# jipolanco/NonuniformFFTs.jl

Measured on AMD Instinct MI355X. Metric: NU-points/s, type-1 NUFFT (set_points! + exec_type1!), 256^3 Float64 m=4, Direct() window (the reference's ROCBackend default), higher is better.
Workload: dtype f64

## Files before the change

nonuniformffts.jl_amd/csrc/balance.hip:

```cpp
#include <hip/hip_runtime.h>

#include <algorithm>
#include <atomic>
#include <hipcub/hipcub.hpp>

#include "device_common.h"
#include "kernels.h"

namespace nufft {

constexpr int kWorkLanes = 16;

__global__ __launch_bounds__(256) void tile_work_kernel(Geom g, int D, int M, const uint32_t* __restrict__ offsets,
                                                       uint32_t* __restrict__ work, const uint32_t* skip_a, const uint32_t* skip_b) {
    if (skip_a && *skip_a != 0u && *skip_b != 0u) return;
    const int nsp = g.sp.ntiles, nip = g.ip.ntiles;
    const int wave = (blockIdx.x * blockDim.x + threadIdx.x) / kWorkLanes;
    const int lane = threadIdx.x & (kWorkLanes - 1);
    if (wave >= nsp + nip) return;
    const bool interp = wave >= nsp;
    const TileShape& ts = interp ? g.ip : g.sp;
    int rem = interp ? wave - nsp : wave, t[3];
    t[0] = rem % ts.nt[0]; rem /= ts.nt[0];
    t[1] = rem % ts.nt[1]; rem /= ts.nt[1];
    t[2] = rem;
    BinSegs seg[3];
    for (int d = 0; d < 3; ++d) {
        seg[d].n = 1; seg[d].lo[0] = 0; seg[d].len[0] = 1; seg[d].lo[1] = 0; seg[d].len[1] = 0;
        if (d >= D) continue;
        const int org = t[d] * ts.n[d];
        const int neff = min(ts.n[d], g.Nover[d] - org);
        if (interp) {
            seg[d].lo[0] = org >> g.blog[d];
            seg[d].len[0] = ((org + neff - 1) >> g.blog[d]) - seg[d].lo[0] + 1;
        } else {
            seg[d] = bin_segments(org - M, org + neff + M - 1, g.Nover[d], g.blog[d], g.nb[d]);
        }
    }
    const int R2 = seg[1].total(), R3 = seg[2].total();
    const int nruns = R2 * R3 * seg[0].n;
    uint32_t sum = 0;
    for (int item = lane; item < nruns; item += kWorkLanes) {
        const int sg = item % seg[0].n;
        const int r2 = (item / seg[0].n) % R2;
        const int r3 = item / (seg[0].n * R2);
        const int bin0 = (seg[2].bin(r3) * g.nb[1] + seg[1].bin(r2)) * g.nb[0] + (sg ? seg[0].lo[1] : seg[0].lo[0]);
        sum += offsets[bin0 + (sg ? seg[0].len[1] : seg[0].len[0])] - offsets[bin0];
    }
    for (int o = kWorkLanes / 2; o > 0; o >>= 1) sum += __shfl_down(sum, o, kWorkLanes);
    if (lane == 0) work[wave] = sum;
}

constexpr int kSumBlocks = 128;

__global__ __launch_bounds__(256) void tile_work_sums_kernel(const uint32_t* __restrict__ work, int nsp, int nip,
                                                            unsigned long long* __restrict__ part, const uint32_t* skip_a, const uint32_t* skip_b) {
    __shared__ unsigned long long wsum[2][256 / kWave];
    if (skip_a && *skip_a != 0u && *skip_b != 0u) return;
    const int tid = threadIdx.x, n = nsp + nip;
    unsigned long long acc[2] = {0ull, 0ull};
    for (int t = blockIdx.x * blockDim.x + tid; t < n; t += gridDim.x * blockDim.x) acc[t >= nsp ? 1 : 0] += work[t];
    for (int k = 0; k < 2; ++k) {
        unsigned long long v = acc[k];
        for (int o = kWave / 2; o > 0; o >>= 1) v += __shfl_down(v, o, kWave);
        if ((tid & (kWave - 1)) == 0) wsum[k][tid / kWave] = v;
    }
    __syncthreads();
    if (tid < 2) {
        unsigned long long v = 0;
        for (int w = 0; w < 256 / kWave; ++w) v += wsum[tid][w];
        part[tid * kSumBlocks + blockIdx.x] = v;
    }
}

__global__ __launch_bounds__(256) void tile_slices_kernel(const uint32_t* __restrict__ work, int nsp, int nip,
                                                         uint32_t extra_sp, uint32_t extra_ip, uint32_t smax,
                                                         const unsigned long long* __restrict__ part,
                                                         uint32_t* __restrict__ nslices, const uint32_t* skip_a, const uint32_t* skip_b) {
    __shared__ unsigned long long tot[2];
    if (skip_a && *skip_a != 0u && *skip_b != 0u) {
        const int t = blockIdx.x * blockDim.x + threadIdx.x;
        if (t < nsp + nip) nslices[t] = 1u;
        return;
    }
    const int tid = threadIdx.x, n = nsp + nip;
    if (tid < 2 * kWave) {
        const int k = tid / kWave, lane = tid & (kWave - 1);
        unsigned long long v = 0;
        for (int b = lane; b < kSumBlocks; b += kWave) v += part[k * kSumBlocks + b];
        for (int o = kWave / 2; o > 0; o >>= 1) v += __shfl_down(v, o, kWave);
        if (lane == 0) tot[k] = v;
    }
    __syncthreads();
    const int t = blockIdx.x * blockDim.x + tid;
    if (t > n) return;
    if (t == n) { nslices[t] = 0; return; }
    const bool interp = t >= nsp;
    const unsigned long long W = tot[interp ? 1 : 0];
    unsigned long long s = W ? (unsigned long long)work[t] * (interp ? extra_ip : extra_sp) / W : 0ull;
    if (s > smax - 1) s = smax - 1;
    nslices[t] = 1u + (uint32_t)s;
}

__global__ __launch_bounds__(256) void fill_desc_kernel(const uint32_t* __restrict__ nslices,
                                                       const uint32_t* __restrict__ desc_off, int nsp, int nip,
                                                       uint32_t ip_base, uint2* __restrict__ desc,
                                                       uint32_t* __restrict__ slots_in_use, const uint32_t* skip_a, const uint32_t* skip_b,
                                                       const uint32_t* sp_served) {
    constexpr int kLanes = 8;
    const int t = (blockIdx.x * blockDim.x + threadIdx.x) / kLanes, lane = threadIdx.x & (kLanes - 1);
    if (skip_a && *skip_a != 0u && *skip_b != 0u) {
        if (blockIdx.x == 0 && threadIdx.x < 2) slots_in_use[threadIdx.x] = 0u;
        return;
    }
    if (t >= nsp + nip) return;
    const uint32_t split = desc_off[nsp];
    const bool interp = t >= nsp;
    const uint32_t S = nslices[t];
    const uint32_t off = interp ? ip_base + (desc_off[t] - split) : desc_off[t];
    const uint32_t tile = interp ? (uint32_t)(t - nsp) : (uint32_t)t;
    for (uint32_t s = lane; s < S; s += kLanes) desc[off + s] = make_uint2(tile, (s << 16) | S);
    if (t == 0 && lane == 0) {
        slots_in_use[0] = (sp_served && *sp_served != 0u) ? 0u : split;
        slots_in_use[1] = desc_off[nsp + nip] - split;
    }
}

size_t balance_work_words(int ntiles_both) {
    return (((size_t)ntiles_both + 1 + 1) & ~(size_t)1) + 4 * (size_t)kSumBlocks;
}

size_t balance_scan_tmp_bytes(int ntiles_both) {
    size_t bytes = 0;
    (void)hipcub::DeviceScan::ExclusiveSum(nullptr, bytes, (uint32_t*)nullptr, (uint32_t*)nullptr, ntiles_both + 1);
    return bytes;
}

hipError_t launch_balance(const BalanceArgs& b, hipStream_t stream) {
    const int nsp = b.g.sp.ntiles, nip = b.g.ip.ntiles, n = nsp + nip;
    const int waves_per_block = 256 / kWorkLanes;
    hipLaunchKernelGGL(tile_work_kernel, dim3((unsigned)((n + waves_per_block - 1) / waves_per_block)), dim3(256), 0, stream,
                       b.g, b.D, b.M, b.offsets, b.work, b.skip_a, b.skip_b);
    unsigned long long* part = reinterpret_cast<unsigned long long*>(b.work + balance_work_words(n) - 4 * kSumBlocks);
    hipLaunchKernelGGL(tile_work_sums_kernel, dim3(kSumBlocks), dim3(256), 0, stream, b.work, nsp, nip, part, b.skip_a, b.skip_b);
    hipLaunchKernelGGL(tile_slices_kernel, dim3((unsigned)((n + 1 + 255) / 256)), dim3(256), 0, stream, b.work, nsp, nip,
                       b.enabled ? b.extra_sp : 0u, b.enabled ? b.extra_ip : 0u, b.smax, part, b.nslices, b.skip_a, b.skip_b);
    size_t tmp = b.scan_tmp_bytes;
    hipError_t e = hipcub::DeviceScan::ExclusiveSum(b.scan_tmp, tmp, b.nslices, b.desc_off, n + 1, stream);
    if (e != hipSuccess) return e;
    hipLaunchKernelGGL(fill_desc_kernel, dim3((unsigned)((n + 31) / 32)), dim3(256), 0, stream, b.nslices, b.desc_off, nsp, nip,
                       (uint32_t)nsp + b.extra_sp, b.desc, b.slots_in_use, b.skip_a, b.skip_b, b.sp_served);
    return hipGetLastError();
}

constexpr int kPatchMaxLayers = 2048;

__global__ __launch_bounds__(256) void patch_column_sums_kernel(Geom g, int npx, int npy, int pbx, int pby, int segl, const uint32_t* __restrict__ offsets,
                                                               uint32_t* __restrict__ colsum, uint32_t* __restrict__ choice) {
    __shared__ uint32_t seg_all[256 / kWave][kPatchMaxLayers];
    const int w = threadIdx.x / kWave, lane = threadIdx.x & (kWave - 1);
    const int c = blockIdx.x * (256 / kWave) + w;
    if (c >= npx * npy) return;
    const int bx0 = (c % npx) * pbx, by0 = (c / npx) * pby;
    const int ncx = min(pbx, g.nb[0] - bx0), ncy = min(pby, g.nb[1] - by0);
    const int nz = g.nb[2], nseg = (nz + segl - 1) / segl;
    uint32_t* seg = seg_all[w];
    for (int s = lane; s < nseg; s += kWave) seg[s] = 0u;
    wave_lds_fence();
    uint32_t total = 0;
    for (int z = lane; z < nz; z += kWave) {
        uint32_t n = 0;
        for (int y = 0; y < ncy; ++y) {
            const int64_t bin0 = ((int64_t)z * g.nb[1] + by0 + y) * g.nb[0] + bx0;
            n += offsets[bin0 + ncx] - offsets[bin0];
        }
        total += n;
        if (n) atomicAdd(&seg[z / segl], n);
    }
    wave_lds_fence();
    uint32_t heaviest = 0;
    for (int s = lane; s < nseg; s += kWave) heaviest = max(heaviest, seg[s]);
    for (int o = kWave / 2; o > 0; o >>= 1) {
        total += __shfl_down(total, o, kWave);
        heaviest = max(heaviest, (uint32_t)__shfl_down(heaviest, o, kWave));
    }
    if (lane == 0) {
        colsum[c] = total;
        atomicMax(&choice[6], heaviest);
    }
}

__global__ __launch_bounds__(1024) void patch_task_counts_kernel(int ncols, int ntasks, int ntab, int nseg, int min_seg, int max_seg, unsigned long long np,
                                                                unsigned long long limit, unsigned long long slots_eff, int uniform_always,
                                                                const uint32_t* __restrict__ colsum, uint32_t* __restrict__ first,
                                                                uint2* __restrict__ tasktab, uint32_t* __restrict__ choice,
                                                                uint32_t* __restrict__ slots_in_use) {
    __shared__ uint32_t part[1024];
    __shared__ uint32_t carry;
    __shared__ int uniform_mode;
    const int tid = threadIdx.x;
    if (tid == 0) {
        carry = 0;
        const double mean = (double)np / (double)ntasks;
        const uint32_t heaviest = choice[6];
        choice[6] = 0u;
        choice[kHaloStateWord] = 0u;
        uniform_mode = (double)heaviest <= 1.1 * mean + 5.0 * sqrt(mean) + 8.0;
        choice[3] = uniform_mode ? 1u : 0u;
        if (uniform_mode) {
            const bool keep = uniform_always || np == 0ull || ((unsigned long long)heaviest <= limit && np <= limit * slots_eff);
            choice[2] = keep ? 1u : 0u;
            if (keep && slots_in_use) slots_in_use[0] = 0u;
        }
    }
    __syncthreads();
    const bool uni = uniform_mode != 0;
    for (int c0 = 0; c0 < ncols; c0 += 1024) {
        const int c = c0 + tid;
        uint32_t S = 0;
        if (c < ncols) {
            if (uni) S = (uint32_t)nseg;
            else {
                S = np ? (uint32_t)(((unsigned long long)ntasks * colsum[c] + np / 2) / np) : 1u;
                S = S < (uint32_t)min_seg ? (uint32_t)min_seg : (S > (uint32_t)max_seg ? (uint32_t)max_seg : S);
            }
        }
        part[tid] = S;
        __syncthreads();
        for (int o = 1; o < 1024; o <<= 1) {
            const uint32_t v = tid >= o ? part[tid - o] : 0u;
            __syncthreads();
            part[tid] += v;
            __syncthreads();
        }
        if (c < ncols) first[c] = carry + part[tid] - S;
        __syncthreads();
        if (tid == 1023) carry += part[1023];
        __syncthreads();
    }
    if (tid == 0) first[ncols] = carry;
    for (int t = (int)carry + tid; t < ntab; t += 1024) tasktab[t] = make_uint2(0u, 0u);
}

__global__ __launch_bounds__(256) void patch_split_kernel(Geom g, int npx, int npy, int pbx, int pby, int clo, int chi, int zq, int segl, int maxlen,
                                                         const uint32_t* __restrict__ offsets, const uint32_t* __restrict__ first,
                                                         unsigned long long limit, unsigned long long limit_cut, unsigned long long slots_eff, int uniform_always,
                                                         double rho_eff_max, unsigned long long np,
                                                         uint2* __restrict__ tasktab, uint32_t* __restrict__ choice,
                                                         uint32_t* __restrict__ slots_in_use) {
    __shared__ uint32_t cum_all[256 / kWave][kPatchMaxLayers + 1];
    __shared__ uint16_t bnd_all[256 / kWave][kPatchMaxLayers + 2];
    const int w = threadIdx.x / kWave, lane = threadIdx.x & (kWave - 1);
    const int c = blockIdx.x * (256 / kWave) + w;
    const int nz = g.nb[2];
    if (choice[3] != 0u) {
        if (c < npx * npy) {
            const uint32_t S = first[c + 1] - first[c];
            for (uint32_t k = lane; k < S; k += kWave) {
                const int z0 = min(nz, (int)k * segl), z1 = min(nz, ((int)k + 1) * segl);
                tasktab[k * (uint32_t)(npx * npy) + (uint32_t)c] = make_uint2((uint32_t)c, z1 > z0 ? ((uint32_t)z1 << 16) | (uint32_t)z0 : 0u);
            }
        }
        return;
    }
    uint32_t* cum = cum_all[w];
    unsigned long long wsum = 0, wsq = 0;
    uint32_t wmax = 0;
    if (c < npx * npy) {
        const int bx0 = (c % npx) * pbx, by0 = (c / npx) * pby;
        const int ncx = min(pbx, g.nb[0] - bx0), ncy = min(pby, g.nb[1] - by0);
        const int per = (nz + kWave - 1) / kWave;
        uint32_t run = 0;
        for (int k = 0; k < per; ++k) {
            const int z = lane * per + k;
            if (z < nz) {
                uint32_t n = 0;
                for (int y = 0; y < ncy; ++y) {
                    const int64_t bin0 = ((int64_t)z * g.nb[1] + by0 + y) * g.nb[0] + bx0;
                    n += offsets[bin0 + ncx] - offsets[bin0];
                }
                run += n;
                wsq += (unsigned long long)n * n;
                cum[z + 1] = run;
            }
        }
        uint32_t incl = run;
        for (int o = 1; o < kWave; o <<= 1) {
            const uint32_t v = __shfl_up(incl, o, kWave);
            if (lane >= o) incl += v;
        }
        const uint32_t before = incl - run;
        for (int k = 0; k < per; ++k) {
            const int z = lane * per + k;
            if (z < nz) cum[z + 1] += before;
        }
        if (lane == 0) cum[0] = 0;
        wave_lds_fence();
        const uint32_t total = cum[nz];
        const uint32_t t0 = first[c], S = first[c + 1] - t0;
        constexpr bool uni = false;
        auto boundary = [&](uint32_t k) -> int {
            if (k == 0) return 0;
            if (k >= S) return nz;
            if (uni) return min(nz, (int)k * segl);
            int z;
            if (total == 0) {
                z = (int)((unsigned long long)k * nz / S);
            } else {
                const uint32_t target = (uint32_t)(((unsigned long long)k * total + S - 1) / S);
                int lo = 0, hi = nz;
                while (lo < hi) {
                    const int mid = (lo + hi) >> 1;
                    if (cum[mid] >= target) hi = mid; else lo = mid + 1;
                }
                z = lo;
            }
            z = (z + zq - 1) / zq * zq;
            return z < nz ? z : nz;
        };
        uint16_t* bnd = bnd_all[w];
        for (uint32_t k = lane; k <= S; k += kWave) bnd[k] = (uint16_t)boundary(k);
        wave_lds_fence();
        if (maxlen > 0 && !uni && lane == 0) {
            for (uint32_t k = 1; k < S; ++k) bnd[k] = (uint16_t)min((int)bnd[k], (int)bnd[k - 1] + maxlen);
            for (int k = (int)S - 1; k > 0; --k) bnd[k] = (uint16_t)max((int)bnd[k], (int)bnd[k + 1] - maxlen);
        }
        wave_lds_fence();
        for (uint32_t k = lane; k < S; k += kWave) {
            const int z0 = bnd[k], z1 = bnd[k + 1];
            tasktab[uni ? k * (uint32_t)(npx * npy) + (uint32_t)c : t0 + k] = make_uint2((uint32_t)c, z1 > z0 ? ((uint32_t)z1 << 16) | (uint32_t)z0 : 0u);
            if (z1 > z0) {
                const uint32_t work = cum[min(nz, z1 - clo)] - cum[max(0, z0 - chi)];
                wsum += work;
                wmax = max(wmax, work);
            }
        }
        for (int o = kWave / 2; o > 0; o >>= 1) {
            wsum += __shfl_down(wsum, o, kWave);
            wsq += __shfl_down(wsq, o, kWave);
            wmax = max(wmax, (uint32_t)__shfl_down(wmax, o, kWave));
        }
        if (lane == 0) {
            atomicMax(&choice[0], wmax);
            atomicAdd(reinterpret_cast<unsigned long long*>(choice + 4), wsum);
            atomicAdd(reinterpret_cast<unsigned long long*>(choice + 8), wsq);
        }
    }
    __syncthreads();
    if (threadIdx.x == 0) {
        __threadfence();
        const uint32_t ticket = atomicAdd(&choice[1], 1u);
        if (ticket == gridDim.x - 1) {
            __threadfence();
            const unsigned long long mx = atomicExch(&choice[0], 0u);
            const unsigned long long sum = atomicExch(reinterpret_cast<unsigned long long*>(choice + 4), 0ull);
            const unsigned long long sumsq = atomicExch(reinterpret_cast<unsigned long long*>(choice + 8), 0ull);
            choice[1] = 0u;
            const unsigned long long lim = choice[3] != 0u ? limit : limit_cut;
            bool patches = (mx <= lim && sum <= lim * slots_eff) || sum == 0ull || (uniform_always && choice[3] != 0u);
            if (rho_eff_max > 0.0 && np > 0ull && !uniform_always) {
                const double rho_eff = (double)sumsq / (double)np / ((double)(pbx * pby) * 64.0);
                if (rho_eff > rho_eff_max) patches = false;
            }
            choice[2] = patches ? 1u : 0u;
            if (patches && slots_in_use) slots_in_use[0] = 0u;
        }
    }
}

constexpr int kPatchSortMax = 16384;

__global__ __launch_bounds__(1024) void patch_task_sort_kernel(int ntasks, int npad, const uint32_t* __restrict__ first, int ncols,
                                                              const uint32_t* __restrict__ choice, uint2* __restrict__ tasktab) {
    extern __shared__ __attribute__((aligned(16))) unsigned char smem_sort[];
    unsigned long long* key = reinterpret_cast<unsigned long long*>(smem_sort);
    const int tid = threadIdx.x;
    if (choice[3] != 0u) return;
    for (int t = tid; t < npad; t += 1024) {
        unsigned long long k = ~0ull;
        if (t < ntasks) {
            const uint2 e = tasktab[t];
            if (e.y != 0u) k = ((unsigned long long)(t - first[e.x]) << 48) | ((unsigned long long)e.x << 32) | e.y;
        }
        key[t] = k;
    }
    __syncthreads();
    for (int size = 2; size <= npad; size <<= 1) {
        for (int stride = size >> 1; stride > 0; stride >>= 1) {
            for (int i = tid; i < npad / 2; i += 1024) {
                const int lo = 2 * i - (i & (stride - 1));
                const int hi = lo + stride;
                const bool up = (lo & size) == 0;
                const unsigned long long a = key[lo], b = key[hi];
                if ((a > b) == up) { key[lo] = b; key[hi] = a; }
            }
            __syncthreads();
        }
    }
    for (int t = tid; t < ntasks; t += 1024) {
        const unsigned long long k = key[t];
        tasktab[t] = k == ~0ull ? make_uint2(0u, 0u) : make_uint2((uint32_t)(k >> 32) & 0xffffu, (uint32_t)k);
    }
}

bool patch_tasks_supported(const Geom& g) { return g.nb[2] <= kPatchMaxLayers; }

hipError_t prepare_column_tasks() {
    return hipFuncSetAttribute(reinterpret_cast<const void*>(patch_task_sort_kernel), hipFuncAttributeMaxDynamicSharedMemorySize, kPatchSortMax * 8);
}
int patch_task_table_entries(const PatchPlan& pp) { return pp.ntasks + 2 * pp.npx * pp.npy; }

static hipError_t launch_column_tasks(const Geom& g, const ColumnTasks& ct, const uint32_t* offsets, int64_t np, unsigned long long limit,
                                      unsigned long long limit_cut, unsigned long long slots_eff, bool uniform_always, uint32_t* choice, uint32_t* slots_in_use,
                                      uint32_t* colsum, uint32_t* first, uint2* tasktab, hipStream_t stream, double rho_eff_max = 0.0) {
    const int ncols = ct.ncolx * ct.ncoly, wpb = 256 / kWave;
    const int ntab = column_task_table_entries(ct, g.nb[2]);
    hipLaunchKernelGGL(patch_column_sums_kernel, dim3((unsigned)((ncols + wpb - 1) / wpb)), dim3(256), 0, stream, g, ct.ncolx, ct.ncoly, ct.bxw, ct.byw,
                       ct.segl, offsets, colsum, choice);
    const int min_seg = ct.maxlen > 0 ? (g.nb[2] + ct.maxlen - 1) / ct.maxlen : 1;
    hipLaunchKernelGGL(patch_task_counts_kernel, dim3(1), dim3(1024), 0, stream, ncols, ct.ntasks, ntab, ct.nseg, min_seg, g.nb[2] / ct.zq,
                       (unsigned long long)np, limit, slots_eff, uniform_always ? 1 : 0, colsum, first, tasktab, choice, slots_in_use);
    hipLaunchKernelGGL(patch_split_kernel, dim3((unsigned)((ncols + wpb - 1) / wpb)), dim3(256), 0, stream, g, ct.ncolx, ct.ncoly, ct.bxw, ct.byw,
                       ct.clo, ct.chi, ct.zq, ct.segl, ct.maxlen, offsets, first, limit, limit_cut, slots_eff, uniform_always ? 1 : 0, rho_eff_max,
                       (unsigned long long)np, tasktab, choice, slots_in_use);
    if (ntab <= kPatchSortMax && ncols < 65536) {
        int npad = 2;
        while (npad < ntab) npad <<= 1;
        hipLaunchKernelGGL(patch_task_sort_kernel, dim3(1), dim3(1024), (size_t)npad * 8, stream, ntab, npad, first, ncols, choice, tasktab);
    }
    return hipGetLastError();
}

hipError_t launch_patch_tasks(const Geom& g, const PatchPlan& pp, int clo, int chi, const uint32_t* offsets, int64_t np,
                              int wave_slots, double advantage, uint32_t* choice, uint32_t* slots_in_use, uint32_t* colsum, uint32_t* first,
                              uint2* tasktab, hipStream_t stream) {
    ColumnTasks ct{pp.npx, pp.npy, 4, pp.pby, pp.nseg, pp.segl, pp.ntasks, pp.f32acc ? 2 : 1, clo, chi, 0};
    const unsigned long long slots_eff = (unsigned long long)std::max(1, std::min(wave_slots, pp.ntasks));
    const double infl0 = (double)(pp.segl + (chi - clo)) / (double)pp.segl;
    const unsigned long long limit = advantage > 0.0 ? (unsigned long long)(advantage * infl0 * (double)np / (double)slots_eff) + 64ull
                                                     : ~0ull / (slots_eff + 1ull);
    return launch_column_tasks(g, ct, offsets, np, limit, limit, slots_eff, true, choice, slots_in_use, colsum, first, tasktab, stream);
}

hipError_t launch_march_tasks(const Geom& g, const ColumnTasks& ct, const uint32_t* offsets, int64_t np, int cus, double advantage, double rho_eff_max,
                              uint32_t* choice, uint32_t* colsum, uint32_t* first, uint2* tasktab, hipStream_t stream) {
    const unsigned long long slots_eff = (unsigned long long)std::max(1, std::min(cus, ct.ntasks));
    const bool always = advantage <= 0.0;
    const unsigned long long limit = always ? ~0ull / (slots_eff + 1ull) : (unsigned long long)(advantage * (double)np / (double)cus) + 64ull;
    const unsigned long long limit_cut = always ? limit : (unsigned long long)(0.85 * advantage * (double)np / (double)cus) + 64ull;
    return launch_column_tasks(g, ct, offsets, np, limit, limit_cut, slots_eff, always, choice, nullptr, colsum, first, tasktab, stream,
                               always ? 0.0 : rho_eff_max);
}

hipError_t launch_smarch_tasks(const Geom& g, const SMarchPlan& sp, const uint32_t* offsets, int64_t np, int cus, double advantage,
                               uint32_t* choice, uint32_t* slots_in_use, uint32_t* colsum, uint32_t* first, uint2* tasktab, hipStream_t stream) {
    const ColumnTasks& ct = sp.ct;
    const unsigned long long slots_eff = (unsigned long long)std::max(1, std::min(cus, ct.ntasks));
    const double infl0 = (double)(ct.segl + sp.hlo + sp.hhi) / (double)ct.segl;
    const unsigned long long limit = advantage > 0.0 ? (unsigned long long)(advantage * infl0 * (double)np / (double)cus) + 64ull
                                                     : ~0ull / (slots_eff + 1ull);
    return launch_column_tasks(g, ct, offsets, np, limit, limit, slots_eff, advantage <= 0.0, choice, slots_in_use, colsum, first, tasktab, stream);
}

template <typename T>
__global__ __launch_bounds__(256) void zero_split_tiles_kernel(Geom g, int D, int ncr, const uint32_t* __restrict__ nslices,
                                                              T* grid, int64_t grid_stride) {
    const TileShape& ts = g.sp;
    const int tile = blockIdx.x;
    if (nslices[tile] <= 1) return;
    T* gr = grid + (int64_t)blockIdx.y * grid_stride;
    int rem = tile, t[3], org[3], neff[3];
    t[0] = rem % ts.nt[0]; rem /= ts.nt[0];
    t[1] = rem % ts.nt[1]; rem /= ts.nt[1];
    t[2] = rem;
    for (int d = 0; d < 3; ++d) {
        org[d] = t[d] * ts.n[d];
        neff[d] = d < D ? min(ts.n[d], g.Nover[d] - org[d]) : 1;
    }
    const int w_row = ncr * neff[0];
    const int rows = neff[1] * neff[2];
    for (int i = threadIdx.x; i < rows * w_row; i += blockDim.x) {
        const int e = i % w_row, r = i / w_row;
        const int l2 = r % neff[1], l3 = r / neff[1];
        int64_t rowbase = 0;
        if (D >= 2) rowbase = org[1] + l2;
        if (D >= 3) rowbase += (int64_t)(org[2] + l3) * g.Nover[1];
        gr[(rowbase * g.Nover[0] + org[0]) * ncr + e] = T(0);
    }
}

hipError_t launch_zero_split_tiles(int dtype, const Geom& g, int D, int is_complex, int C, const uint32_t* nslices,
                                   void* grid, int64_t grid_stride_reals, hipStream_t stream) {
    const dim3 grid_dim((unsigned)g.sp.ntiles, (unsigned)C, 1);
    const int ncr = is_complex ? 2 : 1;
    if (dtype == NUFFT_F32)
        hipLaunchKernelGGL(zero_split_tiles_kernel<float>, grid_dim, dim3(256), 0, stream, g, D, ncr, nslices,
                           static_cast<float*>(grid), grid_stride_reals);
    else
        hipLaunchKernelGGL(zero_split_tiles_kernel<double>, grid_dim, dim3(256), 0, stream, g, D, ncr, nslices,
                           static_cast<double*>(grid), grid_stride_reals);
    return hipGetLastError();
}

}
```

nonuniformffts.jl_amd/csrc/binsort.hip:

```cpp
#include <hip/hip_runtime.h>
#include <hipcub/hipcub.hpp>

#include "device_common.h"
#include "kernels.h"

namespace nufft {

template <typename T, int D>
struct BinArgs {
    const T* x[3];
    int64_t np;
    Geom g;
    int point_transform;
};

template <typename T, int D>
__device__ __forceinline__ uint32_t tile_of_point(const BinArgs<T, D>& a, int64_t p, T (&r)[D]) {
    uint32_t bin = 0, mul = 1;
#pragma unroll
    for (int d = 0; d < D; ++d) {
        const T xf = transform_and_fold(a.x[d][p], a.point_transform);
        r[d] = to_grid_units(xf, a.g.Nover[d]);
        const int i = cell_of(r[d], a.g.Nover[d]);
        bin += mul * (uint32_t)(i >> a.g.blog[d]);
        mul *= (uint32_t)a.g.nb[d];
    }
    return bin;
}

constexpr int kCountThreads = 256;
constexpr int kCountPPT = 4;
constexpr int kCountSlots = 2048;
constexpr uint32_t kEmptyKey = 0xFFFFFFFFu;

template <typename T, int D>
__global__ __launch_bounds__(kCountThreads) void bin_count_kernel(BinArgs<T, D> a, uint32_t* __restrict__ counts,
                                                                 uint2* __restrict__ binrank, const uint32_t* skip_a, const uint32_t* skip_b) {
    __shared__ uint32_t keys[kCountSlots], cnt[kCountSlots], base[kCountSlots];
    if (skip_a && *skip_a != 0u && *skip_b != 0u) return;
    constexpr int kChunkPts = kCountThreads * kCountPPT;
    const int tid = threadIdx.x;
    const int64_t nchunks = (a.np + kChunkPts - 1) / kChunkPts;
    for (int64_t chunk = blockIdx.x; chunk < nchunks; chunk += gridDim.x) {
        for (int s = tid; s < kCountSlots; s += kCountThreads) { keys[s] = kEmptyKey; cnt[s] = 0; }
        __syncthreads();
        uint32_t bin[kCountPPT], lrank[kCountPPT];
        int slot[kCountPPT];
#pragma unroll
        for (int k = 0; k < kCountPPT; ++k) {
            const int64_t p = chunk * kChunkPts + (int64_t)k * kCountThreads + tid;
            slot[k] = -1;
            if (p < a.np) {
                T r[D];
                bin[k] = tile_of_point<T, D>(a, p, r);
                int h = (int)((bin[k] * 2654435761u) >> 21);
                for (;;) {
                    const uint32_t old = atomicCAS(&keys[h], kEmptyKey, bin[k]);
                    if (old == kEmptyKey || old == bin[k]) break;
                    h = (h + 1) & (kCountSlots - 1);
                }
                slot[k] = h;
                lrank[k] = atomicAdd(&cnt[h], 1u);
            }
        }
        __syncthreads();
        for (int s = tid; s < kCountSlots; s += kCountThreads)
            if (keys[s] != kEmptyKey) base[s] = atomicAdd(&counts[keys[s]], cnt[s]);
        __syncthreads();
#pragma unroll
        for (int k = 0; k < kCountPPT; ++k) {
            const int64_t p = chunk * kChunkPts + (int64_t)k * kCountThreads + tid;
            if (slot[k] >= 0) binrank[p] = make_uint2(bin[k], base[slot[k]] + lrank[k]);
        }
        __syncthreads();
    }
}

template <typename T, int D>
__global__ __launch_bounds__(256) void bin_scatter_kernel(BinArgs<T, D> a, const uint32_t* __restrict__ offsets,
                                                         const uint2* __restrict__ binrank,
                                                         PointRec<T, D>* __restrict__ sorted, uint32_t* __restrict__ counts, int ncounts,
                                                         const uint32_t* skip_a, const uint32_t* skip_b) {
    if (skip_a && *skip_a != 0u && *skip_b != 0u) return;
    const int64_t stride = (int64_t)gridDim.x * blockDim.x;
    for (int64_t i = (int64_t)blockIdx.x * blockDim.x + threadIdx.x; i < ncounts; i += stride) counts[i] = 0u;
    for (int64_t p = (int64_t)blockIdx.x * blockDim.x + threadIdx.x; p < a.np; p += stride) {
        const uint2 br = binrank[p];
        PointRec<T, D> rec;
#pragma unroll
        for (int d = 0; d < D; ++d) {
            const T xf = transform_and_fold(a.x[d][p], a.point_transform);
            rec.r[d] = to_grid_units(xf, a.g.Nover[d]);
        }
        rec.idx = (int32_t)p;
        sorted[offsets[br.x] + br.y] = rec;
    }
}

__global__ void zero_fill_kernel(uint4* __restrict__ dst, int64_t n16, uint32_t* __restrict__ tail, int ntail) {
    const int64_t stride = (int64_t)gridDim.x * blockDim.x;
    const int64_t first = (int64_t)blockIdx.x * blockDim.x + threadIdx.x;
    for (int64_t i = first; i < n16; i += stride) dst[i] = make_uint4(0u, 0u, 0u, 0u);
    if (first < ntail) tail[first] = 0u;
}

hipError_t launch_zero_fill(void* dst, size_t bytes, hipStream_t stream) {
    if (bytes == 0) return hipSuccess;
    const int64_t n16 = (int64_t)(bytes / 16);
    const int ntail = (int)((bytes % 16) / 4);
    int64_t blocks = (n16 + 1023) / 1024;
    if (blocks < 1) blocks = 1;
    if (blocks > 256 * 16) blocks = 256 * 16;
    hipLaunchKernelGGL(zero_fill_kernel, dim3((unsigned)blocks), dim3(256), 0, stream, static_cast<uint4*>(dst), n16,
                       reinterpret_cast<uint32_t*>(static_cast<unsigned char*>(dst) + n16 * 16), ntail);
    return hipGetLastError();
}

template <typename T, int D>
static hipError_t run_binsort(const SortArgs& s, hipStream_t stream) {
    BinArgs<T, D> a;
    for (int d = 0; d < 3; ++d) a.x[d] = d < D ? static_cast<const T*>(s.coords[d]) : nullptr;
    a.np = s.np;
    a.g = s.g;
    a.point_transform = s.point_transform;
    hipError_t e = hipSuccess;
    if (!s.counts_clean) {
        e = launch_zero_fill(s.counts, sizeof(uint32_t) * (size_t)(s.g.nbins + 1), stream);
        if (e != hipSuccess) return e;
    }
    if (s.np > 0) {
        int64_t blocks = (s.np + kCountThreads * kCountPPT - 1) / (kCountThreads * kCountPPT);
        if (blocks > 256 * 16) blocks = 256 * 16;
        hipLaunchKernelGGL((bin_count_kernel<T, D>), dim3((unsigned)blocks), dim3(kCountThreads), 0, stream, a, s.counts,
                           static_cast<uint2*>(s.binrank), (const uint32_t*)nullptr, (const uint32_t*)nullptr);
    }
    size_t tmp = s.scan_tmp_bytes;
    e = hipcub::DeviceScan::ExclusiveSum(s.scan_tmp, tmp, s.counts, s.offsets, s.g.nbins + 1, stream);
    if (e != hipSuccess) return e;
    if (s.np > 0) {
        const int threads = 256;
        int64_t blocks = (s.np + threads - 1) / threads;
        if (blocks > 256 * 32) blocks = 256 * 32;
        hipLaunchKernelGGL((bin_scatter_kernel<T, D>), dim3((unsigned)blocks), dim3(threads), 0, stream, a, s.offsets,
                           static_cast<const uint2*>(s.binrank), static_cast<PointRec<T, D>*>(s.sorted), s.counts, s.g.nbins + 1,
                           (const uint32_t*)nullptr, (const uint32_t*)nullptr);
    }
    return hipGetLastError();
}

struct CoarseGeom {
    int cbx, cby, ncx, ncy, nkeys;
};
constexpr int kCoarseThreads = 1024;

template <typename T>
__device__ __forceinline__ uint32_t coarse_key_of(const BinArgs<T, 3>& a, const CoarseGeom& c, const T (&x)[3], T (&r)[3]) {
    int b[3];
#pragma unroll
    for (int d = 0; d < 3; ++d) {
        const T xf = transform_and_fold(x[d], a.point_transform);
        r[d] = to_grid_units(xf, a.g.Nover[d]);
        b[d] = cell_of(r[d], a.g.Nover[d]) >> a.g.blog[d];
    }
    return (uint32_t)((b[2] * c.ncy + b[1] / c.cby) * c.ncx + b[0] / c.cbx);
}
template <typename T, int U>
__device__ __forceinline__ void coarse_load(const BinArgs<T, 3>& a, int64_t p0, int64_t hi, int tid, T (&x)[U][3]) {
#pragma unroll
    for (int u = 0; u < U; ++u) {
        const int64_t p = p0 + u * kCoarseThreads + tid;
        if (p < hi) {
#pragma unroll
            for (int d = 0; d < 3; ++d) x[u][d] = a.x[d][p];
        }
    }
}
__device__ __forceinline__ int64_t coarse_rep_bin(const Geom& g, const CoarseGeom& c, int k) {
    const int cx = k % c.ncx, t = k / c.ncx, cy = t % c.ncy, bz = t / c.ncy;
    return ((int64_t)bz * g.nb[1] + cy * c.cby) * g.nb[0] + cx * c.cbx;
}
__device__ __forceinline__ void coarse_slice(int64_t np, int groups, int w, int64_t& lo, int64_t& hi) {
    int64_t per = (np + groups - 1) / groups;
    per = (per + kCoarseThreads - 1) / kCoarseThreads * kCoarseThreads;
    lo = per * w < np ? per * w : np;
    hi = lo + per < np ? lo + per : np;
}

template <typename T>
__global__ __launch_bounds__(kCoarseThreads) void coarse_count_kernel(BinArgs<T, 3> a, CoarseGeom c, uint32_t* __restrict__ table) {
    extern __shared__ uint32_t hist[];
    const int tid = threadIdx.x, w = blockIdx.x;
    for (int k = tid; k < c.nkeys; k += kCoarseThreads) hist[k] = 0u;
    __syncthreads();
    int64_t lo, hi;
    coarse_slice(a.np, (int)gridDim.x, w, lo, hi);
    constexpr int U = 4;
    constexpr int64_t S = (int64_t)U * kCoarseThreads;
    T xa[U][3], xb[U][3];
    auto consume = [&](int64_t p0, const T (&x)[U][3]) __attribute__((always_inline)) {
#pragma unroll
        for (int u = 0; u < U; ++u) {
            T r[3];
            if (p0 + u * kCoarseThreads + tid < hi) atomicAdd(&hist[coarse_key_of<T>(a, c, x[u], r)], 1u);
        }
    };
    int64_t p0 = lo;
    if (p0 < hi) coarse_load<T, U>(a, p0, hi, tid, xa);
    while (p0 < hi) {
        if (p0 + S < hi) coarse_load<T, U>(a, p0 + S, hi, tid, xb);
        consume(p0, xa);
        p0 += S;
        if (p0 >= hi) break;
        if (p0 + S < hi) coarse_load<T, U>(a, p0 + S, hi, tid, xa);
        consume(p0, xb);
        p0 += S;
    }
    __syncthreads();
    uint32_t* row = table + (size_t)w * c.nkeys;
    for (int k = tid; k < c.nkeys; k += kCoarseThreads) row[k] = hist[k];
}

__global__ __launch_bounds__(64) void coarse_prefix_kernel(Geom g, CoarseGeom c, int groups, uint32_t* __restrict__ table, uint32_t* __restrict__ counts,
                                                            uint32_t* __restrict__ maxout) {
    const int k = blockIdx.x * 64 + threadIdx.x;
    uint32_t run = 0u;
    if (k < c.nkeys) {
    int w = 0;
    for (; w + 8 <= groups; w += 8) {
        uint32_t v[8];
#pragma unroll
        for (int u = 0; u < 8; ++u) v[u] = table[(size_t)(w + u) * c.nkeys + k];
#pragma unroll
        for (int u = 0; u < 8; ++u) {
            table[(size_t)(w + u) * c.nkeys + k] = run;
            run += v[u];
        }
    }
    for (; w < groups; ++w) {
        const uint32_t v = table[(size_t)w * c.nkeys + k];
        table[(size_t)w * c.nkeys + k] = run;
        run += v;
    }
    counts[coarse_rep_bin(g, c, k)] = run;
    }
    if (maxout) {
        uint32_t m = run;
#pragma unroll
        for (int o = 32; o > 0; o >>= 1) m = max(m, (uint32_t)__shfl_xor((int)m, o));
        if (threadIdx.x == 0) atomicMax(maxout, m);
// ... 89 lines not shown
    auto scan_bins = [&]() __attribute__((always_inline)) {
        uint32_t v[4], tsum = 0u;
#pragma unroll
        for (int j = 0; j < 4; ++j) {
            const int i = 4 * tid + j;
            v[j] = i < nbs ? cnt[i] : 0u;
            tsum += v[j];
        }
        uint32_t incl = tsum;
#pragma unroll
        for (int o = 1; o < 64; o <<= 1) {
            const uint32_t t = (uint32_t)__shfl_up((int)incl, o);
            if (lane >= o) incl += t;
        }
        if (lane == 63) wsum[wave] = incl;
        __syncthreads();
        uint32_t wbase = 0u;
        for (int w = 0; w < wave; ++w) wbase += wsum[w];
        uint32_t run = wbase + incl - tsum;
#pragma unroll
        for (int j = 0; j < 4; ++j) {
            const int i = 4 * tid + j;
            if (i < nbs) {
                cnt[i] = run;
                offsets[rep + i] = base + run;
            }
            run += v[j];
        }
        __syncthreads();
    };
    auto bin_of = [&](const PointRec<T, 3>& rec) __attribute__((always_inline)) -> uint32_t {
        const int b0 = cell_of(rec.r[0], g.Nover[0]) >> g.blog[0], b1 = cell_of(rec.r[1], g.Nover[1]) >> g.blog[1];
        return (uint32_t)((b1 - cy * c.cby) * g.nb[0] + b0);
    };
    if (n > (uint32_t)cap) {
        for (uint32_t i = (uint32_t)tid; i < n; i += kSlabThreads) atomicAdd(&cnt[bin_of(temp[base + i])], 1u);
        __syncthreads();
        scan_bins();
        for (uint32_t i = (uint32_t)tid; i < n; i += kSlabThreads) {
            const PointRec<T, 3> rec = temp[base + i];
            sorted[base + atomicAdd(&cnt[bin_of(rec)], 1u)] = rec;
        }
        return;
    }
    uint32_t av[kSlabIPT];
#pragma unroll
    for (int u = 0; u < kSlabIPT; ++u) {
        const uint32_t i = (uint32_t)(u * kSlabThreads + tid);
        av[u] = 0u;
        if (i < n) {
            const PointRec<T, 3> rec = temp[base + i];
            recs[i] = rec;
            const uint32_t fb = bin_of(rec);
            av[u] = fb << 16 | atomicAdd(&cnt[fb], 1u);
        }
    }
    __syncthreads();
    scan_bins();
#pragma unroll
    for (int u = 0; u < kSlabIPT; ++u) {
        const uint32_t i = (uint32_t)(u * kSlabThreads + tid);
        if (i < n) aux[cnt[av[u] >> 16] + (av[u] & 0xffffu)] = i;
    }
    __syncthreads();
    for (uint32_t j = (uint32_t)tid; j < n; j += kSlabThreads) sorted[base + j] = recs[aux[j]];
}

static CoarseGeom coarse_geom(const CoarseSort& cs) { return CoarseGeom{cs.cbx, cs.cby, cs.ncx, cs.ncy, cs.nkeys}; }

template <typename T>
static BinArgs<T, 3> bin_args3(const SortArgs& s) {
    BinArgs<T, 3> a;
    for (int d = 0; d < 3; ++d) a.x[d] = static_cast<const T*>(s.coords[d]);
    a.np = s.np;
    a.g = s.g;
    a.point_transform = s.point_transform;
    return a;
}

int slab_sort_lds_bytes(int dtype, int cap) {
    return (kSlabMaxBins + 16) * 4 + cap * (4 + (int)(dtype == NUFFT_F32 ? sizeof(PointRec<float, 3>) : sizeof(PointRec<double, 3>)));
}
int slab_sort_capacity(int dtype, int lds_bytes) {
    const int rb = 4 + (int)(dtype == NUFFT_F32 ? sizeof(PointRec<float, 3>) : sizeof(PointRec<double, 3>));
    int cap = (lds_bytes - (kSlabMaxBins + 16) * 4) / rb;
    cap &= ~63;
    return cap > kSlabIPT * kSlabThreads ? kSlabIPT * kSlabThreads : cap;
}
hipError_t prepare_binsort_slab(int dtype, int lds_bytes) {
    hipError_t e = prepare_binsort_coarse(dtype, kCoarseMaxKeys);
    if (e != hipSuccess) return e;
    return dtype == NUFFT_F32 ? hipFuncSetAttribute(reinterpret_cast<const void*>(&slab_sort_kernel<float>), hipFuncAttributeMaxDynamicSharedMemorySize, lds_bytes)
                              : hipFuncSetAttribute(reinterpret_cast<const void*>(&slab_sort_kernel<double>), hipFuncAttributeMaxDynamicSharedMemorySize, lds_bytes);
}
hipError_t prepare_binsort_coarse(int dtype, int nkeys) {
    if (nkeys > kCoarseMaxKeys) return hipErrorInvalidValue;
    const int bytes = kCoarseMaxKeys * 4;
    hipError_t e;
    if (dtype == NUFFT_F32) {
        e = hipFuncSetAttribute(reinterpret_cast<const void*>(&coarse_count_kernel<float>), hipFuncAttributeMaxDynamicSharedMemorySize, bytes);
        if (e == hipSuccess) e = hipFuncSetAttribute(reinterpret_cast<const void*>(&coarse_scatter_kernel<float>), hipFuncAttributeMaxDynamicSharedMemorySize, bytes);
    } else {
        e = hipFuncSetAttribute(reinterpret_cast<const void*>(&coarse_count_kernel<double>), hipFuncAttributeMaxDynamicSharedMemorySize, bytes);
        if (e == hipSuccess) e = hipFuncSetAttribute(reinterpret_cast<const void*>(&coarse_scatter_kernel<double>), hipFuncAttributeMaxDynamicSharedMemorySize, bytes);
    }
    return e;
}

template <typename T>
static hipError_t coarse_count_t(const SortArgs& s, hipStream_t stream) {
    const CoarseGeom c = coarse_geom(s.cs);
    hipError_t e = hipSuccess;
    if (!s.counts_clean) {
        e = launch_zero_fill(s.counts, sizeof(uint32_t) * (size_t)(s.g.nbins + 1), stream);
        if (e != hipSuccess) return e;
    }
    hipLaunchKernelGGL((coarse_count_kernel<T>), dim3((unsigned)s.cs.groups), dim3(kCoarseThreads), (size_t)c.nkeys * 4, stream, bin_args3<T>(s), c, s.cs.table);
    hipLaunchKernelGGL(coarse_prefix_kernel, dim3((unsigned)((c.nkeys + 63) / 64)), dim3(64), 0, stream, s.g, c, s.cs.groups, s.cs.table, s.counts,
                       s.cs.mode == 2 ? s.cs.flagmem : (uint32_t*)nullptr);
    if (s.cs.mode == 2) hipLaunchKernelGGL(slab_flag_kernel, dim3(1), dim3(1), 0, stream, s.cs.flagmem, (uint32_t)s.cs.cap * (uint32_t)kSlabOverfill);
    size_t tmp = s.scan_tmp_bytes;
    return hipcub::DeviceScan::ExclusiveSum(s.scan_tmp, tmp, s.counts, s.offsets, s.g.nbins + 1, stream);
}

template <typename T>
static hipError_t coarse_finish_t(const SortArgs& s, hipStream_t stream) {
    const CoarseGeom c = coarse_geom(s.cs);
    const BinArgs<T, 3> a = bin_args3<T>(s);
    const uint32_t *fa = s.cs.flag_a, *fb = s.cs.flag_b;
    hipLaunchKernelGGL(coarse_clear_kernel, dim3((unsigned)((c.nkeys + 255) / 256)), dim3(256), 0, stream, s.g, c, s.counts, fa, fb);
    if (s.np > 0) {
        int64_t blocks = (s.np + kCountThreads * kCountPPT - 1) / (kCountThreads * kCountPPT);
        if (blocks > 256 * 16) blocks = 256 * 16;
        hipLaunchKernelGGL((bin_count_kernel<T, 3>), dim3((unsigned)blocks), dim3(kCountThreads), 0, stream, a, s.counts, static_cast<uint2*>(s.binrank), fa, fb);
    }
    size_t tmp = s.scan_tmp_bytes;
    hipError_t e = hipcub::DeviceScan::ExclusiveSum(s.scan_tmp, tmp, s.counts, s.offsets, s.g.nbins + 1, stream);
    if (e != hipSuccess) return e;
    hipLaunchKernelGGL((coarse_scatter_kernel<T>), dim3((unsigned)s.cs.groups), dim3(kCoarseThreads), (size_t)c.nkeys * 4, stream, a, c, s.cs.table, s.offsets,
                       static_cast<PointRec<T, 3>*>(s.cs.mode == 2 ? s.cs.temp : s.sorted), s.counts, fa, fb, s.cs.fb_a, s.cs.fb_b,
                       (s.cs.fb_a && s.cs.fb_b) ? s.cs.feedback : (uint32_t*)nullptr, s.cs.seq);
    if (s.cs.mode == 2)
        hipLaunchKernelGGL((slab_sort_kernel<T>), dim3((unsigned)c.nkeys), dim3(kSlabThreads), (size_t)s.cs.lds2, stream, s.g, c, s.cs.cap,
                           static_cast<const PointRec<T, 3>*>(s.cs.temp), static_cast<PointRec<T, 3>*>(s.sorted), s.offsets, fa);
    if (s.np > 0) {
        int64_t blocks = (s.np + 255) / 256;
        if (blocks > 256 * 32) blocks = 256 * 32;
        hipLaunchKernelGGL((bin_scatter_kernel<T, 3>), dim3((unsigned)blocks), dim3(256), 0, stream, a, s.offsets, static_cast<const uint2*>(s.binrank),
                           static_cast<PointRec<T, 3>*>(s.sorted), s.counts, s.g.nbins + 1, fa, fb);
    }
    return hipGetLastError();
}

__global__ void sort_feedback_kernel(const uint32_t* ra, const uint32_t* rb, uint32_t* feedback, uint32_t seq) {
    __atomic_store_n(&feedback[0], *ra, __ATOMIC_RELAXED);
    __atomic_store_n(&feedback[1], *rb, __ATOMIC_RELAXED);
    __threadfence_system();
    __atomic_store_n(&feedback[2], seq, __ATOMIC_RELAXED);
}
hipError_t launch_sort_feedback(const uint32_t* ra, const uint32_t* rb, uint32_t* feedback, uint32_t seq, hipStream_t stream) {
    hipLaunchKernelGGL(sort_feedback_kernel, dim3(1), dim3(1), 0, stream, ra, rb, feedback, seq);
    return hipGetLastError();
}

hipError_t launch_binsort_coarse_count(const SortArgs& s, hipStream_t stream) {
    return s.dtype == NUFFT_F32 ? coarse_count_t<float>(s, stream) : coarse_count_t<double>(s, stream);
}
hipError_t launch_binsort_coarse_finish(const SortArgs& s, hipStream_t stream) {
    return s.dtype == NUFFT_F32 ? coarse_finish_t<float>(s, stream) : coarse_finish_t<double>(s, stream);
}

size_t binsort_scan_tmp_bytes(int nbins) {
    size_t bytes = 0;
    uint32_t* p = nullptr;
    (void)hipcub::DeviceScan::ExclusiveSum(nullptr, bytes, p, p, nbins + 1, (hipStream_t)0);
    return bytes < 16 ? 16 : bytes;
}

size_t point_record_bytes(int dtype, int D) {
    if (dtype == NUFFT_F32) return D == 1 ? sizeof(PointRec<float, 1>) : D == 2 ? sizeof(PointRec<float, 2>) : sizeof(PointRec<float, 3>);
    return D == 1 ? sizeof(PointRec<double, 1>) : D == 2 ? sizeof(PointRec<double, 2>) : sizeof(PointRec<double, 3>);
}

hipError_t launch_binsort(const SortArgs& s, hipStream_t stream) {
    if (s.dtype == NUFFT_F32) {
        switch (s.D) {
            case 1: return run_binsort<float, 1>(s, stream);
            case 2: return run_binsort<float, 2>(s, stream);
            default: return run_binsort<float, 3>(s, stream);
        }
    }
    switch (s.D) {
        case 1: return run_binsort<double, 1>(s, stream);
        case 2: return run_binsort<double, 2>(s, stream);
        default: return run_binsort<double, 3>(s, stream);
    }
}

template <int REC_BYTES>
__global__ void extract_perm_kernel(const unsigned char* __restrict__ recs, int idx_off, int64_t np, int32_t* __restrict__ perm) {
    const int64_t p = (int64_t)blockIdx.x * blockDim.x + threadIdx.x;
    if (p < np) perm[p] = *reinterpret_cast<const int32_t*>(recs + p * REC_BYTES + idx_off);
}

hipError_t launch_extract_perm(int dtype, int D, const void* sorted, int64_t np, int32_t* perm_dev, hipStream_t stream) {
    if (np <= 0) return hipSuccess;
    const size_t rb = point_record_bytes(dtype, D);
    const int idx_off = D * (dtype == NUFFT_F32 ? 4 : 8);
    const unsigned blocks = (unsigned)((np + 255) / 256);
    const unsigned char* r = static_cast<const unsigned char*>(sorted);
    switch (rb) {
        case 8: hipLaunchKernelGGL(extract_perm_kernel<8>, dim3(blocks), dim3(256), 0, stream, r, idx_off, np, perm_dev); break;
        case 16: hipLaunchKernelGGL(extract_perm_kernel<16>, dim3(blocks), dim3(256), 0, stream, r, idx_off, np, perm_dev); break;
        default: hipLaunchKernelGGL(extract_perm_kernel<32>, dim3(blocks), dim3(256), 0, stream, r, idx_off, np, perm_dev); break;
    }
    return hipGetLastError();
}

}
```

nonuniformffts.jl_amd/csrc/column_tasks.h:

```cpp
#pragma once

#include <cstdint>

#if defined(__HIPCC__)
#define NUFFT_HD __host__ __device__
#else
#define NUFFT_HD
#endif

namespace nufft {

struct ColumnTasks {
    int ncolx, ncoly, bxw, byw, nseg, segl, ntasks, zq, clo, chi, maxlen;
};

inline int column_task_table_entries(const ColumnTasks& ct, int nz) {
    const int min_seg = ct.maxlen > 0 ? (nz + ct.maxlen - 1) / ct.maxlen : 1;
    return ct.ntasks + (min_seg + 1) * ct.ncolx * ct.ncoly;
}

struct SMarchPlan {
    bool eligible;
    int n1, n2;
    int hlo, hhi;
    int halo;
    int64_t halo_reals;
    int parts;
    int lds_bytes, threads;
    ColumnTasks ct;
    double visits, efficiency;
};

struct HaloLayout {
    int n1, n2, xlo, xhi, ylo, yhi, nc;
    int ntx, nty;
    int sw, rw, rec;
    int64_t plane;
};
NUFFT_HD inline HaloLayout make_halo_layout(int n1, int n2, int M, int nc, int ntx, int nty) {
    HaloLayout h;
    h.n1 = n1; h.n2 = n2; h.nc = nc; h.ntx = ntx; h.nty = nty;
    h.xlo = (M - 1) + ((M - 1) & 1); h.xhi = M; h.ylo = M - 1; h.yhi = M;
    h.sw = ((h.xlo + h.xhi) * nc + 1) & ~1;
    h.rw = ((n1 + h.xlo + h.xhi) * nc + 1) & ~1;
    h.rec = n2 * h.sw + (h.ylo + h.yhi) * h.rw;
    h.plane = (int64_t)h.rec * ntx * nty;
    return h;
}
NUFFT_HD inline int halo_record_offset(const HaloLayout& h, int lxw, int ly) {
    if (ly < 0) return h.n2 * h.sw + (ly + h.ylo) * h.rw + lxw;
    if (ly >= h.n2) return h.n2 * h.sw + (h.ylo + ly - h.n2) * h.rw + lxw;
    return ly * h.sw + (lxw < h.xlo * h.nc ? lxw : lxw - h.n1 * h.nc);
}

struct CoarseSort {
    int enabled;
    int cbx, cby, ncx, ncy;
    int nkeys;
    int groups;
    uint32_t* table;
    const uint32_t* flag_a;
    const uint32_t* flag_b;
    int mode;
    void* temp;
    int cap, lds2;
    uint32_t* flagmem;
    const uint32_t* fb_a;
    const uint32_t* fb_b;
    uint32_t* feedback;
    uint32_t seq;
};
constexpr int kSlabMaxBins = 4096;
constexpr int kHaloStateWord = 12;
constexpr int kSlabOverfill = 8;
constexpr int kCoarseMaxKeys = 36864;

}
```

nonuniformffts.jl_amd/csrc/kernels.h:

```cpp
#pragma once

#include "options.h"
#include <hip/hip_runtime.h>
#include <cstdint>

#include "column_tasks.h"
#include "device_common.h"
#include "nufft_mi355x.h"

namespace nufft {

struct SortArgs {
    CoarseSort cs;
    int dtype, D;
    int point_transform;
    int64_t np;
    const void* coords[3];
    Geom g;
    uint32_t* counts;
    bool counts_clean;
    uint32_t* offsets;
    void* binrank;
    void* sorted;
    void* scan_tmp;
    size_t scan_tmp_bytes;
};
size_t binsort_scan_tmp_bytes(int nbins);
size_t point_record_bytes(int dtype, int D);
hipError_t launch_binsort(const SortArgs& s, hipStream_t stream);
hipError_t prepare_binsort_coarse(int dtype, int nkeys);
int slab_sort_capacity(int dtype, int lds_bytes);
int slab_sort_lds_bytes(int dtype, int cap);
hipError_t prepare_binsort_slab(int dtype, int lds_bytes);
hipError_t launch_binsort_coarse_count(const SortArgs& s, hipStream_t stream);
hipError_t launch_binsort_coarse_finish(const SortArgs& s, hipStream_t stream);
hipError_t launch_sort_feedback(const uint32_t* ra, const uint32_t* rb, uint32_t* feedback, uint32_t seq, hipStream_t stream);
hipError_t launch_zero_fill(void* dst, size_t bytes, hipStream_t stream);
hipError_t launch_extract_perm(int dtype, int D, const void* sorted, int64_t np, int32_t* perm_dev, hipStream_t stream);

struct BalanceArgs {
    Geom g;
    int D, M;
    bool enabled;
    uint32_t extra_sp, extra_ip;
    uint32_t smax;
    const uint32_t* offsets;
    uint32_t* work;
    uint32_t* nslices;
    uint32_t* desc_off;
    uint2* desc;
    uint32_t* slots_in_use;
    void* scan_tmp;
    size_t scan_tmp_bytes;
    const uint32_t* skip_a;
    const uint32_t* skip_b;
    const uint32_t* sp_served;
};
size_t balance_scan_tmp_bytes(int ntiles_both);
size_t balance_work_words(int ntiles_both);
hipError_t launch_balance(const BalanceArgs& b, hipStream_t stream);
hipError_t launch_zero_split_tiles(int dtype, const Geom& g, int D, int is_complex, int C, const uint32_t* nslices,
                                   void* grid, int64_t grid_stride_reals, hipStream_t stream);


struct TileKernelArgs {
    int dtype, is_complex, D, M, evalmode, C;
    int kernel;
    Geom g;
    const void* sorted;
    const uint32_t* offsets;
    const void* coefs;
    double beta[3];
    double beta_over_pi[3];
    void* grid;
    int64_t grid_stride;
    const void* const* values_in;
    void* const* values_out;
    double prefactor;
    const void* weights;
    int threads;
    int lds_bytes;
    int ntiles;
    const void* desc;
    const uint32_t* desc_total;
    int xcd_chunk;
    int march;
    ColumnTasks march_ct;
    const uint32_t* march_flag;
    const uint2* march_tasks;
    int fixed_tile;
    int cubes;
    void* halo;
    int interp_parts;
    int coarse;
    const uint32_t* coarse_a;
    const uint32_t* coarse_b;
};
void interp_fixed_dims(int dtype, int is_complex, int D, int M, int* n);
void spread_fixed_dims(int dtype, int is_complex, int D, int M, int* n);
bool spread_cubes_available(int dtype, int is_complex, int D, int M);
bool interp_march_available(int dtype, int is_complex, int D, int M, bool poly, const Geom& g, bool other);
hipError_t prepare_interp_march(int dtype, int is_complex, int M, bool poly);
bool interp_march_staged_available(int dtype, int is_complex, int M, bool poly, int n1, int n2);
hipError_t prepare_interp_march_staged(int dtype, int is_complex, int M, bool poly);
ColumnTasks march_column_tasks(int dtype, int is_complex, int M, bool poly, const Geom& g, int n1 = 0, int n2 = 0);
hipError_t launch_spread(const TileKernelArgs& a, hipStream_t stream);
hipError_t launch_interp(const TileKernelArgs& a, hipStream_t stream);
hipError_t prepare_spread(int dtype, int is_complex, int D, int M, int lds_bytes, bool other);
hipError_t prepare_interp(int dtype, int is_complex, int D, int M, int lds_bytes, bool other);
bool needs_other_eval(int kernel, int evalmode);

struct PatchPlan {
    bool eligible;
    int npx, npy, nseg, segl, ntasks;
    int lds_bytes;
    int pby;
    int occ;
    int f32acc;
    int planar;
};
PatchPlan patch_plan(int dtype, int is_complex, int D, int M, const Geom& g, bool other, bool allow_f32acc = true, int planar_nc = 0);
hipError_t launch_march_tasks(const Geom& g, const ColumnTasks& ct, const uint32_t* offsets, int64_t np, int cus, double advantage, double rho_eff_max,
                              uint32_t* choice, uint32_t* colsum, uint32_t* first, uint2* tasktab, hipStream_t stream);
hipError_t launch_patch_tasks(const Geom& g, const PatchPlan& pp, int clo, int chi, const uint32_t* offsets, int64_t np,
                              int wave_slots, double advantage, uint32_t* choice, uint32_t* slots_in_use, uint32_t* colsum, uint32_t* first,
                              uint2* tasktab, hipStream_t stream);
bool patch_tasks_supported(const Geom& g);
hipError_t prepare_column_tasks();
int patch_task_table_entries(const PatchPlan& pp);
hipError_t prepare_spread_patch(int dtype, int is_complex, int M, bool other, int planar_nc = 0);
hipError_t launch_gather_planar(int dtype, int D, const void* sorted, int64_t np, const void* const* vin, int C,
                                const void* weights, void* vout, const uint32_t* enabled, hipStream_t stream);
hipError_t launch_spread_patch(const TileKernelArgs& a, const PatchPlan& pp, const void* vsorted, int64_t vstride_reals,
                               const uint32_t* enabled, const uint2* tasktab, hipStream_t stream);
hipError_t launch_gather_values(int dtype, int is_complex, int D, const void* sorted, int64_t np, const void* vin,
                                const void* weights, void* vout, const uint32_t* enabled, hipStream_t stream);

SMarchPlan smarch_plan(int dtype, int is_complex, int D, int M, const Geom& g, bool other, int cus, int C, int halo, int parts = 1);
hipError_t prepare_spread_march(int dtype, int is_complex, int M, int halo);
hipError_t launch_spread_march(const TileKernelArgs& a, const SMarchPlan& sp, const uint32_t* flag, const uint2* tasktab, uint32_t* halo_state, bool dense, hipStream_t stream);
bool spread_dense_available(int dtype, int is_complex, int M, bool poly, const SMarchPlan& sp);
hipError_t prepare_spread_dense(int dtype, int M, bool poly);
hipError_t launch_smarch_halo_add(const TileKernelArgs& a, const SMarchPlan& sp, const uint32_t* flag, hipStream_t stream);
hipError_t launch_smarch_tasks(const Geom& g, const SMarchPlan& sp, const uint32_t* offsets, int64_t np, int cus, double advantage,
                               uint32_t* choice, uint32_t* slots_in_use, uint32_t* colsum, uint32_t* first, uint2* tasktab, hipStream_t stream);

struct GradLaunchArgs {
    int dtype, is_complex, D, M, C;
    int kernel, evalmode;
    int Nover[3];
    const void* sorted;
    int64_t np;
    const void* coefs;
    double p0[3], p1[3];
    const void* grid;
    int64_t grid_stride;
    void* const* values_out;
    void* const* grad_out;
    double prefactor;
    double dscale[3];
};
inline int grad_window_select(int kernel, int evalmode) {
    if (kernel == NUFFT_KERNEL_BACKWARDS_KAISER_BESSEL && evalmode == NUFFT_EVAL_DIRECT) return 0;
    if (evalmode != NUFFT_EVAL_DIRECT && (kernel == NUFFT_KERNEL_BACKWARDS_KAISER_BESSEL || kernel == NUFFT_KERNEL_KAISER_BESSEL)) return 1;
    return 2;
}
hipError_t launch_interp_grad_f32r(const GradLaunchArgs& a, hipStream_t stream);
hipError_t launch_interp_grad_f32c(const GradLaunchArgs& a, hipStream_t stream);
hipError_t launch_interp_grad_f64r(const GradLaunchArgs& a, hipStream_t stream);
hipError_t launch_interp_grad_f64c(const GradLaunchArgs& a, hipStream_t stream);
inline hipError_t launch_interp_grad(const GradLaunchArgs& a, hipStream_t stream) {
    if (a.dtype == NUFFT_F32) return a.is_complex ? launch_interp_grad_f32c(a, stream) : launch_interp_grad_f32r(a, stream);
    return a.is_complex ? launch_interp_grad_f64c(a, stream) : launch_interp_grad_f64r(a, stream);
}

struct DeconvArgs {
    int dtype, D, C;
    int nout[3];
    int nspec[3];
    const void* phihat[3];
    const int32_t* index_map[3];
    const int32_t* inv_map[3];
    void* spec;
    int64_t spec_stride;
    double normfactor;
    const void* mode_factors;
};
hipError_t launch_deconv_truncate(const DeconvArgs& a, void* const* uhat_out, hipStream_t stream);
hipError_t launch_deconv_pad(const DeconvArgs& a, const void* const* uhat_in, hipStream_t stream);

struct FftLinePass {
    const void* in;
    void* out;
    int64_t a_total, a_out;
    int64_t in_stride_j, in_stride_c;
    int64_t out_stride_j, out_stride_c;
    int nc, nk;
    const int32_t* map;
    const void* fa; int ka;
    const void* fk;
    const void* twiddle;
    double scale;
    const void* mult;
    int row_a = 0, row_valid = 0, row_in = 0, row_out = 0;
};
bool fft_lines_supported(int dtype, int64_t n);
bool real_lines_supported(int dtype, int64_t n);
struct RealLineHalo {
    const void* buffer;
    const void* buffer2;
    const uint32_t* flag;
    int ny;
    HaloLayout layout;
};
hipError_t launch_real_lines(int dtype, int64_t n, bool forward, const void* in, void* out, int64_t nlines, int k1, int row,
                             const void* twiddle, hipStream_t stream, const RealLineHalo* halo = nullptr);
hipError_t launch_fft_lines(int dtype, int64_t n, bool forward, const FftLinePass& p, hipStream_t stream);
hipError_t launch_halo_add_lines(int dtype, void* grid, const void* halo, int64_t grid_comp_reals, int64_t halo_comp_reals, int n1cells, int ny, int nz,
                                 int C, const HaloLayout& h, const uint32_t* flag, hipStream_t stream, bool planar = false);
hipError_t launch_cplx_lines(int dtype, int64_t n, bool forward, const void* in, void* out, int64_t nlines, int k1,
                             const int32_t* map, const void* twiddle, hipStream_t stream, const RealLineHalo* halo = nullptr);

}
```

nonuniformffts.jl_amd/csrc/nufft_internal.h:

```cpp
#pragma once

#include "options.h"
#include <cstdint>
#include <map>
#include <string>
#include <utility>
#include <vector>

#include "column_tasks.h"
#include "nufft_mi355x.h"

struct rocfft_plan_t;
struct rocfft_execution_info_t;

namespace nufft {

constexpr int kMaxDim = 3;
constexpr int kMinM = 2;
constexpr int kMaxM = 10;
constexpr int kLdsLimit = 163840;

void set_error(const std::string& msg);

int64_t nextprod235(int64_t n);
// ... 29 lines not shown
    int nb[kMaxDim] = {1, 1, 1};
    int64_t nbins = 1;
    TileShapeHost sp;
    TileShapeHost ip;
};

bool choose_tiles(int D, int M, int ncomp, int real_bytes, const int64_t* Nover, int lds_budget_bytes,
                  int spread_waves, int interp_waves, const int* forced_sp, const int* forced_ip, int bin_log2,
                  TileGeom& g);


}

struct nufft_plan {
    std::map<void*, std::pair<std::string, int64_t>> allocs;
    std::string opts_text;
    nufft::Options opts;
    int dtype = NUFFT_F64;
    bool is_complex = false;
    int D = 1;
    int64_t N[3] = {1, 1, 1};
    int M = 4;
    double sigma_req = 2.0;
    int evalmode = NUFFT_EVAL_DIRECT;
    int C = 1;
    bool fftshift = false;
    int device = -1;
    int spread_threads = 256;
    int interp_threads = 256;

    int64_t Nover[3] = {1, 1, 1};
    int64_t Nout[3] = {1, 1, 1};
    int64_t Nspec[3] = {1, 1, 1};
    double sigma = 2.0;
    double beta[3] = {0, 0, 0};
    const void* cb_point_weights = nullptr;
    const void* cb_mode_factors = nullptr;
    const void* cb_sticky_weights = nullptr;
    const void* cb_sticky_factors = nullptr;
    int kernel = 0;
    int point_transform = 0;
    double tau[3] = {0, 0, 0};
    double eval_p0[3] = {0, 0, 0};
    int scale_exp[3] = {0, 0, 0};
    double beta_over_pi_scaled[3] = {0, 0, 0};
    int npoly = 8;
    std::vector<double> coefs[3];
    std::vector<double> phihat[3];
    std::vector<int64_t> index_map[3];
    nufft::TileGeom tile;
    bool interp_march = false;
    int interp_march_mode = 1;
    bool debug_tasks = false;
    nufft::ColumnTasks march_ct{};
    int num_cus = 256;
    uint32_t* d_march_choice = nullptr;
    uint32_t* d_march_cols = nullptr;
    void* d_march_tasks = nullptr;
    bool interp_fixed = false;
    bool spread_fixed = false;
    bool spread_cubes = false;
    int spread_method = NUFFT_SPREAD_LDS_TILES;
    int spread_method_req = NUFFT_SPREAD_AUTO;
    struct Patch {
        bool eligible = false;
        int npx = 0, npy = 0, nseg = 0, segl = 0, ntasks = 0, lds_bytes = 0, pby = 0, occ = 2, f32acc = 0, planar = 0;
    } patch;
    uint32_t* d_patch_choice = nullptr;
    uint32_t* d_patch_cols = nullptr;
    void* d_patch_tasks = nullptr;
    int interp_parts = 1;
    int smarch_parts = 1;
    nufft::SMarchPlan smarch{};
    uint32_t* d_smarch_choice = nullptr;
    uint32_t* d_smarch_cols = nullptr;
    void* d_smarch_tasks = nullptr;
    void* d_smarch_halo = nullptr;
    bool halo_hint = false;
    bool halo_sticky = false;
    bool halo_fuse = true;
    int wave_slots = 2048;
    void* d_vsorted = nullptr;
    int64_t lds_spread = 0, lds_interp = 0;

    void* d_coefs = nullptr;
    void* d_phihat[3] = {nullptr, nullptr, nullptr};
    int32_t* d_index_map[3] = {nullptr, nullptr, nullptr};
    int32_t* d_inv_map[3] = {nullptr, nullptr, nullptr};
    void* d_us = nullptr;
    void* d_uhat = nullptr;
    int64_t grid_elems = 0;
    int64_t spec_elems = 0;
    int64_t pspec_elems = 0;

    int64_t Np = -1;
    int64_t Np_capacity = 0;
    int64_t binrank_capacity = 0;
    uint32_t* d_counts = nullptr;
    bool counts_clean = false;
    uint32_t* d_offsets = nullptr;
    nufft::CoarseSort slab{};
    int slab_fill = 85;
    int64_t slab_min_points = 0;
    uint32_t* sort_feedback = nullptr;
    uint32_t sort_seq = 0, sort_seq_seen = 0;
    int sort_miss_streak = 0;
    bool sort_prefer_slab = false;
    bool coarse_now = false;
    bool dense_available = false;
    bool dense_now = false;
    int dense_min = 1 << 30;
    int sort_column_pred[2] = {0, 0};
    int slab_max_keys = 0;
    nufft::CoarseSort coarse{};
    void* d_binrank = nullptr;
    void* d_sorted = nullptr;
    void* d_scan_tmp = nullptr;
    size_t scan_tmp_bytes = 0;
    struct Balance {
        uint32_t extra[2] = {0, 0};
        uint32_t* d_work = nullptr;
        uint32_t* d_nslices = nullptr;
        uint32_t* d_desc_off = nullptr;
        void* d_desc = nullptr;
        uint32_t* d_slots = nullptr;
        void* d_tmp = nullptr;
        size_t tmp_bytes = 0;
    } bal;
    bool balance_enabled = true;
    int64_t workspace_bytes = 0;

    bool pruned_fft = false;
    bool compact_dim1 = false;
    int64_t spec_row = 0;
    rocfft_plan_t* fft1_fw = nullptr;
    rocfft_plan_t* fft1_bw = nullptr;
    void* d_tmp2 = nullptr;
    void* d_tw_fw[3] = {nullptr, nullptr, nullptr};
    void* d_tw_bw[3] = {nullptr, nullptr, nullptr};
    void* d_invphi[3] = {nullptr, nullptr, nullptr};
    void* d_one = nullptr;

    rocfft_plan_t* fft_fw = nullptr;
    rocfft_plan_t* fft_bw = nullptr;
    rocfft_execution_info_t* fft_info = nullptr;
    void* d_fft_work = nullptr;
    size_t fft_work_bytes = 0;

    bool timing = false;
    void* ev_begin[NUFFT_NUM_STAGES] = {};
    void* ev_end[NUFFT_NUM_STAGES] = {};
    bool ev_valid[NUFFT_NUM_STAGES] = {};
};
```

nonuniformffts.jl_amd/csrc/plan.cpp:

```cpp
#include <hip/hip_runtime.h>
#include <rocfft/rocfft.h>

#include <algorithm>
#include <cmath>
#include <cstdio>
#include <cstdlib>
#include <cstring>
#include <mutex>
#include <new>
#include <string>

#include "kernels.h"
#include "nufft_internal.h"

namespace nufft {

static thread_local std::string g_last_error;
void set_error(const std::string& msg) { g_last_error = msg; }

static int fail(int code, const std::string& msg) {
    set_error(msg);
    return code;
}

// ... 497 lines not shown
            NUFFT_ROCFFT(rocfft_plan_create(&p->fft_fw, rocfft_placement_notinplace, rocfft_transform_type_real_forward, prec,
                                            (size_t)D, lengths, (size_t)p->C, nullptr));
            NUFFT_ROCFFT(rocfft_plan_create(&p->fft_bw, rocfft_placement_notinplace, rocfft_transform_type_real_inverse, prec,
                                            (size_t)D, lengths, (size_t)p->C, nullptr));
        }
        size_t wf = 0, wb = 0;
        NUFFT_ROCFFT(rocfft_plan_get_work_buffer_size(p->fft_fw, &wf));
        NUFFT_ROCFFT(rocfft_plan_get_work_buffer_size(p->fft_bw, &wb));
        p->fft_work_bytes = std::max(wf, wb);
        if (p->fft_work_bytes > 0) {
            if ((rc = dev_alloc(p, &p->d_fft_work, p->fft_work_bytes, "rocfft_work"))) return rc;
            NUFFT_ROCFFT(rocfft_execution_info_set_work_buffer(p->fft_info, p->d_fft_work, p->fft_work_bytes));
        }
    }

    if (p->pruned_fft && !p->is_complex && !p->compact_dim1) {
        size_t len1[1] = {(size_t)p->Nover[0]};
        size_t batch = (size_t)p->C;
        for (int d = 1; d < D; ++d) batch *= (size_t)p->Nover[d];
        NUFFT_ROCFFT(rocfft_plan_create(&p->fft1_fw, rocfft_placement_notinplace, rocfft_transform_type_real_forward, prec, 1, len1, batch, nullptr));
        NUFFT_ROCFFT(rocfft_plan_create(&p->fft1_bw, rocfft_placement_notinplace, rocfft_transform_type_real_inverse, prec, 1, len1, batch, nullptr));
        size_t w1 = 0, w2 = 0;
        NUFFT_ROCFFT(rocfft_plan_get_work_buffer_size(p->fft1_fw, &w1));
        NUFFT_ROCFFT(rocfft_plan_get_work_buffer_size(p->fft1_bw, &w2));
        if (std::max(w1, w2) > p->fft_work_bytes) {
            dev_free(p, p->d_fft_work);
            p->fft_work_bytes = std::max(w1, w2);
            if ((rc = dev_alloc(p, &p->d_fft_work, p->fft_work_bytes, "rocfft_work"))) return rc;
            NUFFT_ROCFFT(rocfft_execution_info_set_work_buffer(p->fft_info, p->d_fft_work, p->fft_work_bytes));
        }
    }
    if (p->pruned_fft) {
        for (int d = 0; d < D; ++d) {
            std::vector<double> inv(p->phihat[d].size());
            for (size_t i = 0; i < inv.size(); ++i) {
                const double v = p->dtype == NUFFT_F32 ? (double)(float)p->phihat[d][i] : p->phihat[d][i];
                inv[i] = 1.0 / std::ldexp(v, p->scale_exp[d]);
            }
            rc = p->dtype == NUFFT_F32 ? upload<float>(p, &p->d_invphi[d], inv) : upload<double>(p, &p->d_invphi[d], inv);
            if (rc) return rc;
        }
        {
            std::vector<double> one(1, 1.0);
            rc = p->dtype == NUFFT_F32 ? upload<float>(p, &p->d_one, one) : upload<double>(p, &p->d_one, one);
            if (rc) return rc;
        }
        for (int d = p->compact_dim1 ? 0 : 1; d < D; ++d) {
            const int64_t n = p->Nover[d];
            std::vector<double> twf(2 * (size_t)n), twb(2 * (size_t)n);
            for (int64_t m = 0; m < n; ++m) {
                const double ang = 2.0 * M_PI * (double)m / (double)n;
                twf[2 * m] = std::cos(ang); twf[2 * m + 1] = -std::sin(ang);
                twb[2 * m] = std::cos(ang); twb[2 * m + 1] = std::sin(ang);
            }
            rc = p->dtype == NUFFT_F32 ? upload<float>(p, &p->d_tw_fw[d], twf) : upload<double>(p, &p->d_tw_fw[d], twf);
            if (rc) return rc;
            rc = p->dtype == NUFFT_F32 ? upload<float>(p, &p->d_tw_bw[d], twb) : upload<double>(p, &p->d_tw_bw[d], twb);
            if (rc) return rc;
        }
        if (D == 3) {
            const size_t elems = (size_t)(p->compact_dim1 ? p->spec_row : p->Nout[0]) * p->Nout[1] * p->Nover[2];
            if ((rc = dev_alloc(p, &p->d_tmp2, elems * 2 * real_bytes(p), "tmp2"))) return rc;
        }
    }

    for (int other = 0; other < 2; ++other) {
        if (!other && needs_other_eval(p->kernel, p->evalmode)) continue;
        NUFFT_HIP(prepare_spread(p->dtype, p->is_complex, D, p->M, (int)p->lds_spread, other != 0));
        NUFFT_HIP(prepare_interp(p->dtype, p->is_complex, D, p->M, (int)p->lds_interp, other != 0));
    }

    p->debug_tasks = env_int("NUFFT_DEBUG_TASKS", 0) != 0;
    p->halo_fuse = env_int("NUFFT_SMARCH_HALO_FUSE", 1) != 0;
    p->interp_march = choose_interp_ring(p);
    auto march_cplx = [&]() { return p->interp_parts == 2 ? 0 : (int)p->is_complex; };
    if (p->interp_march) {
        NUFFT_HIP(prepare_interp_march(p->dtype, march_cplx(), p->M, p->evalmode != NUFFT_EVAL_DIRECT));
        p->march_ct = march_column_tasks(p->dtype, march_cplx(), p->M, p->evalmode != NUFFT_EVAL_DIRECT, make_geom(p));
        const size_t ncols = (size_t)p->march_ct.ncolx * p->march_ct.ncoly;
        if (ncols >= 65536 || p->tile.nb[2] > 2048) p->interp_march = false;
        else {
            if ((rc = dev_alloc(p, reinterpret_cast<void**>(&p->d_march_choice), 16 * sizeof(uint32_t)))) return rc;
            NUFFT_HIP(hipMemset(p->d_march_choice, 0, 16 * sizeof(uint32_t)));
            if ((rc = dev_alloc(p, reinterpret_cast<void**>(&p->d_march_cols), (2 * ncols + 2) * sizeof(uint32_t)))) return rc;
            if ((rc = dev_alloc(p, &p->d_march_tasks, (size_t)column_task_table_entries(p->march_ct, p->tile.nb[2]) * 8))) return rc;
        }
    }

    if (p->spread_method == NUFFT_SPREAD_MARCHING_RING) {
        const bool other = needs_other_eval(p->kernel, p->evalmode);
        int want_halo = p->smarch.halo;
        if (want_halo == 2 && !(p->pruned_fft && p->compact_dim1) && env_int("NUFFT_SMARCH_HALO", 0) != 2) want_halo = 0;
        for (;;) {
            p->smarch = smarch_plan(p->dtype, p->is_complex, D, p->M, make_geom(p), other, p->num_cus, p->C, want_halo, p->smarch_parts);
            if (!p->smarch.eligible && want_halo)
                p->smarch = smarch_plan(p->dtype, p->is_complex, D, p->M, make_geom(p), other, p->num_cus, p->C, 0, p->smarch_parts);
            if (!p->smarch.eligible || p->smarch.halo != 2) break;
            const size_t bytes = (size_t)p->smarch.halo_reals * real_bytes(p) * p->C * p->smarch.parts;
            if (!env_int("NUFFT_TEST_HALO_ALLOC_FAIL", 0) && dev_alloc(p, &p->d_smarch_halo, bytes, "ring_side_buffer") == NUFFT_OK) break;
            p->d_smarch_halo = nullptr;
            want_halo = 0;
        }
        const int ring_max_m = ring_max_half_support(p);
        const bool keep = p->smarch.eligible && (p->spread_method_req == NUFFT_SPREAD_MARCHING_RING || p->M <= ring_max_m);
        if (!keep) {
            if (p->spread_method_req == NUFFT_SPREAD_MARCHING_RING)
                return fail(NUFFT_ERR_UNSUPPORTED, "marching-ring spreading: no decomposition for this device");
            dev_free(p, p->d_smarch_halo);
            p->smarch.eligible = false;
            const bool prefer_patches = p->is_complex || p->M >= 5 || p->patch.planar != 0;
            p->spread_method = (p->patch.eligible && prefer_patches) ? NUFFT_SPREAD_MFMA_PATCHES : NUFFT_SPREAD_LDS_TILES;
        }
    }
    if (p->spread_method == NUFFT_SPREAD_MARCHING_RING) {
        NUFFT_HIP(prepare_spread_march(p->dtype, p->smarch.parts == 2 ? 0 : p->is_complex, p->M, p->smarch.halo));
        const size_t ncols = (size_t)p->smarch.ct.ncolx * p->smarch.ct.ncoly;
        if ((rc = dev_alloc(p, reinterpret_cast<void**>(&p->d_smarch_choice), 16 * sizeof(uint32_t)))) return rc;
        NUFFT_HIP(hipMemset(p->d_smarch_choice, 0, 16 * sizeof(uint32_t)));
        if ((rc = dev_alloc(p, reinterpret_cast<void**>(&p->d_smarch_cols), (2 * ncols + 2) * sizeof(uint32_t)))) return rc;
        if ((rc = dev_alloc(p, &p->d_smarch_tasks, (size_t)column_task_table_entries(p->smarch.ct, p->tile.nb[2]) * 8))) return rc;
    }

    if (p->spread_method == NUFFT_SPREAD_MFMA_PATCHES) {
        NUFFT_HIP(prepare_spread_patch(p->dtype, p->is_complex, p->M, false, p->patch.planar));
        if ((rc = dev_alloc(p, reinterpret_cast<void**>(&p->d_patch_choice), 16 * sizeof(uint32_t)))) return rc;
        NUFFT_HIP(hipMemset(p->d_patch_choice, 0, 16 * sizeof(uint32_t)));
        const size_t ncols = (size_t)p->patch.npx * p->patch.npy;
        if ((rc = dev_alloc(p, reinterpret_cast<void**>(&p->d_patch_cols), (2 * ncols + 2) * sizeof(uint32_t)))) return rc;
        if ((rc = dev_alloc(p, &p->d_patch_tasks, ((size_t)p->patch.ntasks + 2 * ncols) * 8))) return rc;
        p->wave_slots = p->num_cus * 4 * p->patch.occ;
    }

    p->coarse = CoarseSort{};
    if (p->spread_method == NUFFT_SPREAD_MARCHING_RING && p->smarch.halo == 2 && p->interp_march && D == 3 && env_int("NUFFT_COARSE_SORT", 1) != 0) {
        ColumnTasks shared{};
        const bool same = shared_ring_column(p, p->smarch, &shared);
        const int nkeys = p->smarch.ct.ncolx * p->smarch.ct.ncoly * p->tile.nb[2];
        const int mcplx = p->interp_parts == 2 ? 0 : (int)p->is_complex;
        if (same) {
            p->march_ct = shared;
            const ColumnTasks& mc = p->march_ct;
            const size_t ncols = (size_t)mc.ncolx * mc.ncoly;
            dev_free(p, p->d_march_cols);
            dev_free(p, p->d_march_tasks);
            if ((rc = dev_alloc(p, reinterpret_cast<void**>(&p->d_march_cols), (2 * ncols + 2) * sizeof(uint32_t)))) return rc;
            if ((rc = dev_alloc(p, &p->d_march_tasks, (size_t)column_task_table_entries(mc, p->tile.nb[2]) * 8))) return rc;
            p->coarse.enabled = 1;
            p->coarse.cbx = mc.bxw; p->coarse.cby = mc.byw; p->coarse.ncx = mc.ncolx; p->coarse.ncy = mc.ncoly;
            p->coarse.nkeys = nkeys;
            p->coarse.groups = p->num_cus;
            p->coarse.flag_a = p->d_smarch_choice + 2;
            p->coarse.flag_b = p->d_march_choice + 2;
            if ((rc = dev_alloc(p, reinterpret_cast<void**>(&p->coarse.table), (size_t)p->coarse.groups * nkeys * sizeof(uint32_t), "sort_slice_table"))) return rc;
            NUFFT_HIP(prepare_binsort_coarse(p->dtype, nkeys));
            NUFFT_HIP(prepare_interp_march_staged(p->dtype, mcplx, p->M, p->evalmode != NUFFT_EVAL_DIRECT));
        }
    }

    p->dense_available = p->spread_method == NUFFT_SPREAD_MARCHING_RING && env_int("NUFFT_DENSE", 1) != 0 && !needs_other_eval(p->kernel, p->evalmode) &&
                         spread_dense_available(p->dtype, p->is_complex, p->M, p->evalmode != NUFFT_EVAL_DIRECT, p->smarch);
    if (p->dense_available) NUFFT_HIP(prepare_spread_dense(p->dtype, p->M, p->evalmode != NUFFT_EVAL_DIRECT));
    static const int dense_min_direct[7] = {0, 0, 1 << 30, 1 << 30, 96, 16, 12};
    static const int dense_min_poly[7] = {0, 0, 1 << 30, 1 << 30, 24, 10, 6};
    p->dense_min = env_int("NUFFT_DENSE_MIN", p->M <= 6 ? (p->evalmode == NUFFT_EVAL_DIRECT ? dense_min_direct : dense_min_poly)[p->M] : 1 << 30);

    p->slab = CoarseSort{};
    if (D == 3 && env_int("NUFFT_SLAB_SORT", 1) != 0 && p->tile.nb[0] <= kSlabMaxBins && p->tile.nb[2] <= kCoarseMaxKeys) {
        p->slab.enabled = 1;
        p->slab.mode = 2;
        p->slab_min_points = env_int("NUFFT_SLAB_MIN_POINTS", 16384);
        p->slab_fill = std::min(95, std::max(5, env_int("NUFFT_SLAB_FILL", 85)));
        p->slab_max_keys = (int)std::min<int64_t>(kCoarseMaxKeys, (int64_t)p->tile.nb[1] * p->tile.nb[2]);
        if ((rc = dev_alloc(p, reinterpret_cast<void**>(&p->slab.table), (size_t)p->num_cus * p->slab_max_keys * sizeof(uint32_t), "sort_slice_table"))) return rc;
        if ((rc = dev_alloc(p, reinterpret_cast<void**>(&p->slab.flagmem), 32))) return rc;
        NUFFT_HIP(hipMemset(p->slab.flagmem, 0, 32));
        p->slab.flag_a = p->slab.flag_b = p->slab.flagmem + 4;
        NUFFT_HIP(prepare_binsort_slab(p->dtype, kLdsLimit - 256));
    }

    if (p->coarse.enabled && p->slab.enabled && env_int("NUFFT_SORT_ADAPTIVE", 1) != 0) {
        NUFFT_HIP(hipHostMalloc(reinterpret_cast<void**>(&p->sort_feedback), 16, hipHostMallocMapped));
        p->sort_feedback[0] = p->sort_feedback[1] = 1u;
        p->sort_feedback[2] = 0u;
    }
    if (p->spread_method == NUFFT_SPREAD_MFMA_PATCHES || p->spread_method == NUFFT_SPREAD_MARCHING_RING || p->interp_march) NUFFT_HIP(prepare_column_tasks());

    for (int s = 0; s < NUFFT_NUM_STAGES; ++s) {
        hipEvent_t a, b;
        NUFFT_HIP(hipEventCreate(&a));
        NUFFT_HIP(hipEventCreate(&b));
        p->ev_begin[s] = a;
        p->ev_end[s] = b;
    }
    return NUFFT_OK;
}

static void release(nufft_plan* p) {
    if (!p) return;
    if (current_options() == &p->opts) set_current_options(nullptr);
    if (p->device >= 0) {
        DeviceGuard guard(p->device);
        (void)hipDeviceSynchronize();
        if (p->sort_feedback) (void)hipHostFree(p->sort_feedback);
        for (auto& al : p->allocs) (void)hipFree(al.first);
        p->allocs.clear();
        if (p->fft1_fw) (void)rocfft_plan_destroy(p->fft1_fw);
        if (p->fft1_bw) (void)rocfft_plan_destroy(p->fft1_bw);
        if (p->fft_fw) (void)rocfft_plan_destroy(p->fft_fw);
        if (p->fft_bw) (void)rocfft_plan_destroy(p->fft_bw);
        if (p->fft_info) (void)rocfft_execution_info_destroy(p->fft_info);
        for (int s = 0; s < NUFFT_NUM_STAGES; ++s) {
            if (p->ev_begin[s]) (void)hipEventDestroy(static_cast<hipEvent_t>(p->ev_begin[s]));
            if (p->ev_end[s]) (void)hipEventDestroy(static_cast<hipEvent_t>(p->ev_end[s]));
        }
    }
    delete p;
}

static int require_device(const nufft_plan* p) {
    if (!p) return fail(NUFFT_ERR_INVALID_ARG, "null plan");
    set_current_options(&p->opts);
    if (p->device < 0) return fail(NUFFT_ERR_NO_DEVICE, "host-only plan (device = -1) has no device path");
    return NUFFT_OK;
}

static int require_points(const nufft_plan* p) {
    int rc = require_device(p);
    if (rc) return rc;
    if (p->Np < 0) return fail(NUFFT_ERR_NO_POINTS, "set_points must be called before exec");
    return NUFFT_OK;
}

static TileKernelArgs tile_args(const nufft_plan* p, bool interp) {
    TileKernelArgs a{};
    a.dtype = p->dtype;
    a.is_complex = p->is_complex;
    a.D = p->D;
    a.M = p->M;
    a.evalmode = p->evalmode;
    a.kernel = p->kernel;
    a.C = p->C;
    a.g = make_geom(p);
    a.sorted = p->d_sorted;
    a.offsets = p->d_offsets;
    a.coefs = p->d_coefs;
    for (int d = 0; d < 3; ++d) {
        a.beta[d] = p->eval_p0[d];
        a.beta_over_pi[d] = p->beta_over_pi_scaled[d];
    }
    a.grid = p->d_us;
    a.grid_stride = p->grid_elems;
    a.prefactor = 1.0;
    if (interp) {
        for (int d = 0; d < p->D; ++d) a.prefactor *= 2.0 * M_PI / (double)p->Nover[d];
    }
    a.weights = p->cb_point_weights;
    a.threads = interp ? p->interp_threads : p->spread_threads;
    a.fixed_tile = interp ? p->interp_fixed : p->spread_fixed;
    a.march = interp && p->interp_march;
    a.interp_parts = p->interp_parts;
    a.coarse = p->coarse_now;
    a.coarse_a = p->coarse.flag_a;
    a.coarse_b = p->coarse.flag_b;
    a.march_ct = p->march_ct;
    a.march_flag = p->d_march_choice ? p->d_march_choice + 2 : nullptr;
    a.march_tasks = static_cast<const uint2*>(p->d_march_tasks);
    a.cubes = !interp && p->spread_cubes && !needs_other_eval(p->kernel, p->evalmode) && !p->cb_point_weights;
    a.halo = p->d_smarch_halo;
    a.lds_bytes = (int)(interp ? p->lds_interp : p->lds_spread);
    const nufft_plan::Balance& b = p->bal;
    const int nt = (int)(interp ? p->tile.ip.ntiles : p->tile.sp.ntiles);
    a.ntiles = nt + (int)b.extra[interp ? 1 : 0];
    a.desc = static_cast<const char*>(b.d_desc) + (interp ? ((size_t)p->tile.sp.ntiles + b.extra[0]) * 8 : 0);
    a.desc_total = b.d_slots + (interp ? 1 : 0);
    a.xcd_chunk = env_int("NUFFT_XCD_CHUNK", 8);
    return a;
}

static bool halo_plan(const nufft_plan* p) { return p->spread_method == NUFFT_SPREAD_MARCHING_RING && p->smarch.halo == 2 && p->d_smarch_halo && p->d_smarch_choice; }
static void note_capture(nufft_plan* p, hipStream_t stream) {
    if (p->halo_sticky || !halo_plan(p)) return;
    hipStreamCaptureStatus st = hipStreamCaptureStatusNone;
    if (hipStreamIsCapturing(stream, &st) != hipSuccess) { (void)hipGetLastError(); return; }
    if (st != hipStreamCaptureStatusNone) p->halo_sticky = true;
}
static bool halo_maybe_pending(const nufft_plan* p) { return halo_plan(p) && (p->halo_hint || p->halo_sticky); }
static int void_halo(nufft_plan* p, hipStream_t stream) {
    if (halo_maybe_pending(p)) NUFFT_HIP(launch_zero_fill(p->d_smarch_choice + kHaloStateWord, 4, stream));
    p->halo_hint = false;
    return NUFFT_OK;
}

static int complete_halo(nufft_plan* p, hipStream_t stream) {
    if (!halo_maybe_pending(p)) return NUFFT_OK;
    TileKernelArgs a = tile_args(p, false);
    NUFFT_HIP(launch_smarch_halo_add(a, p->smarch, p->d_smarch_choice + kHaloStateWord, stream));
    NUFFT_HIP(launch_zero_fill(p->d_smarch_choice + kHaloStateWord, 4, stream));
    p->halo_hint = false;
    return NUFFT_OK;
}


static DeconvArgs deconv_args(const nufft_plan* p) {
    DeconvArgs a{};
    a.dtype = p->dtype;
    a.D = p->D;
// ... 313 lines not shown
    o->ring_segments = ring ? p->smarch.ct.nseg : 0;
    o->ring_halo = (ring && p->smarch.halo == 2) ? 1 : 0;
    o->sort_column[0] = p->device < 0 ? p->sort_column_pred[0] : (p->coarse.enabled ? p->coarse.cbx : 0);
    o->sort_column[1] = p->device < 0 ? p->sort_column_pred[1] : (p->coarse.enabled ? p->coarse.cby : 0);
    return NUFFT_OK;
}

int nufft_plan_get_phi_hat(const nufft_plan* p, int dim, double* out, int64_t capacity) {
    if (!p || !out || dim < 0 || dim >= p->D) return fail(NUFFT_ERR_INVALID_ARG, "bad argument");
    if (capacity < (int64_t)p->phihat[dim].size()) return fail(NUFFT_ERR_DIM_MISMATCH, "buffer too small");
    std::memcpy(out, p->phihat[dim].data(), p->phihat[dim].size() * sizeof(double));
    return NUFFT_OK;
}

int nufft_plan_get_poly_coefs(const nufft_plan* p, int dim, double* out, int64_t capacity) {
    if (!p || !out || dim < 0 || dim >= p->D) return fail(NUFFT_ERR_INVALID_ARG, "bad argument");
    if (capacity < (int64_t)p->coefs[dim].size()) return fail(NUFFT_ERR_DIM_MISMATCH, "buffer too small");
    std::memcpy(out, p->coefs[dim].data(), p->coefs[dim].size() * sizeof(double));
    return NUFFT_OK;
}

int nufft_plan_get_index_map(const nufft_plan* p, int dim, int64_t* out, int64_t capacity) {
    if (!p || !out || dim < 0 || dim >= p->D) return fail(NUFFT_ERR_INVALID_ARG, "bad argument");
    if (capacity < (int64_t)p->index_map[dim].size()) return fail(NUFFT_ERR_DIM_MISMATCH, "buffer too small");
    std::memcpy(out, p->index_map[dim].data(), p->index_map[dim].size() * sizeof(int64_t));
    return NUFFT_OK;
}

static int64_t binrank_bytes(const nufft_plan* p, bool slab_sort) {
    return slab_sort ? std::max<int64_t>(8, (int64_t)point_record_bytes(p->dtype, p->D)) : 8;
}

int nufft_set_points(nufft_plan* p, int64_t np, const void* const* coords, void* stream_) {
    int rc = require_device(p);
    if (rc) return rc;
    if (np < 0) return fail(NUFFT_ERR_INVALID_ARG, "negative number of points");
    if (np >= ((int64_t)1 << 31) - 1) return fail(NUFFT_ERR_UNSUPPORTED, "number of points exceeds 2^31 - 2");
    if (!coords) return fail(NUFFT_ERR_INVALID_ARG, "null coordinate table");
    for (int d = 0; d < p->D; ++d)
        if (np > 0 && !coords[d]) return fail(NUFFT_ERR_INVALID_ARG, "null coordinate vector");
    DeviceGuard guard(p->device);
    hipStream_t stream = static_cast<hipStream_t>(stream_);
    p->Np = -1;
    if (np > p->Np_capacity) {
        dev_free(p, p->d_sorted);
        dev_free(p, p->d_vsorted);
        p->Np_capacity = 0;
        if (p->spread_method == NUFFT_SPREAD_MFMA_PATCHES && (rc = dev_alloc(p, &p->d_vsorted, (size_t)np * value_bytes(p) * p->C, "vsorted"))) return rc;
        if ((rc = dev_alloc(p, &p->d_sorted, (size_t)np * point_record_bytes(p->dtype, p->D), "sorted"))) return rc;
        p->Np_capacity = np;
    }
    p->dense_now = p->dense_available && np >= (int64_t)p->dense_min * p->tile.nbins;
    {
        if (p->sort_feedback) {
            hipStreamCaptureStatus st = hipStreamCaptureStatusNone;
            const bool capturing = hipStreamIsCapturing(stream, &st) == hipSuccess && st != hipStreamCaptureStatusNone;
            if (!capturing) (void)hipGetLastError();
            const uint32_t seq = __atomic_load_n(&p->sort_feedback[2], __ATOMIC_ACQUIRE);
            if (!capturing && seq != p->sort_seq_seen && seq == p->sort_seq) {
                p->sort_seq_seen = seq;
                const bool both = p->sort_feedback[0] != 0u && p->sort_feedback[1] != 0u;
                if (both) { p->sort_miss_streak = 0; p->sort_prefer_slab = false; }
                else if (++p->sort_miss_streak >= 2) p->sort_prefer_slab = true;
            }
        }
        p->coarse_now = p->coarse.enabled && !p->dense_now && !(p->sort_prefer_slab && p->slab.enabled);
        const bool slab_scratch = p->slab.enabled && !p->coarse_now;
        const int64_t need = np * binrank_bytes(p, slab_scratch);
        if (need > p->binrank_capacity) {
            dev_free(p, p->d_binrank);
            p->binrank_capacity = 0;
            if ((rc = dev_alloc(p, &p->d_binrank, (size_t)need, "sort_scratch"))) return rc;
            p->binrank_capacity = need;
        }
    }
    note_capture(p, stream);
    p->halo_hint = false;
    StageTimer tm(p, NUFFT_STAGE_SET_POINTS, stream);
    SortArgs s{};
    s.dtype = p->dtype;
    s.D = p->D;
    s.point_transform = p->point_transform;
    s.np = np;
    for (int d = 0; d < 3; ++d) s.coords[d] = d < p->D ? coords[d] : nullptr;
    s.g = make_geom(p);
    s.counts = p->d_counts;
    s.counts_clean = p->counts_clean;
    p->counts_clean = false;
    s.offsets = p->d_offsets;
    s.binrank = p->d_binrank;
    s.sorted = p->d_sorted;
    s.scan_tmp = p->d_scan_tmp;
    s.scan_tmp_bytes = p->scan_tmp_bytes;
    s.cs = p->coarse;
    const bool coarse = p->coarse_now;
    if (p->coarse.enabled && !coarse) s.cs = CoarseSort{};
    if (coarse && p->sort_feedback) {
        s.cs.fb_a = p->coarse.flag_a; s.cs.fb_b = p->coarse.flag_b;
        s.cs.feedback = p->sort_feedback; s.cs.seq = ++p->sort_seq;
    }
    bool slab = false;
    if (!coarse && p->slab.enabled && np >= std::max<int64_t>(p->slab_min_points, 1)) {
        const int capmax = slab_sort_capacity(p->dtype, kLdsLimit - 256);
        int best = -1;
        for (int sby = 1; sby <= p->tile.nb[1] && (int64_t)sby * p->tile.nb[0] <= kSlabMaxBins; sby *= 2) {
            const int64_t nkeys = (int64_t)p->tile.nb[2] * ((p->tile.nb[1] + sby - 1) / sby);
            if (nkeys > p->slab_max_keys) continue;
            if (np / nkeys > (int64_t)capmax * p->slab_fill / 100) break;
            if (best > 0 && nkeys < 2048) break;
            best = sby;
        }
        if (best > 0) {
            slab = true;
            s.cs = p->slab;
            s.cs.cbx = p->tile.nb[0]; s.cs.ncx = 1;
            s.cs.cby = best; s.cs.ncy = (p->tile.nb[1] + best - 1) / best;
            s.cs.nkeys = p->tile.nb[2] * s.cs.ncy;
            s.cs.groups = (int)std::min<int64_t>(p->num_cus, std::max<int64_t>(1, (np + 16383) / 16384));
            const int64_t mean = np / s.cs.nkeys;
            s.cs.cap = (int)std::min<int64_t>(capmax, (std::max<int64_t>(2 * mean, mean + 1536) + 63) / 64 * 64);
            s.cs.lds2 = slab_sort_lds_bytes(p->dtype, s.cs.cap);
            s.cs.temp = p->d_binrank;
        }
    }
    if (coarse) NUFFT_HIP(launch_binsort_coarse_count(s, stream));
    else if (slab) {
        NUFFT_HIP(launch_binsort_coarse_count(s, stream));
        NUFFT_HIP(launch_binsort_coarse_finish(s, stream));
    } else {
        if (p->slab.enabled) NUFFT_HIP(launch_zero_fill(p->slab.flagmem + 4, 16, stream));
        NUFFT_HIP(launch_binsort(s, stream));
    }
    auto balance = [&]() -> int {
        const nufft_plan::Balance& b = p->bal;
        BalanceArgs q{};
        q.g = s.g;
        q.D = p->D;
        q.M = p->M;
        q.enabled = p->balance_enabled && np > 0;
        q.extra_sp = b.extra[0];
        q.extra_ip = b.extra[1];
        q.smax = 4096;
        q.offsets = p->d_offsets;
        q.work = b.d_work;
        q.nslices = b.d_nslices;
        q.desc_off = b.d_desc_off;
        q.desc = static_cast<uint2*>(b.d_desc);
        q.slots_in_use = b.d_slots;
        q.scan_tmp = b.d_tmp;
        q.scan_tmp_bytes = b.tmp_bytes;
        q.skip_a = coarse ? p->coarse.flag_a : nullptr;
        q.skip_b = coarse ? p->coarse.flag_b : nullptr;
        q.sp_served = coarse ? p->coarse.flag_a : nullptr;
        NUFFT_HIP(launch_balance(q, stream));
        return NUFFT_OK;
    };
    if (!coarse && (rc = balance())) return rc;
    if (p->spread_method == NUFFT_SPREAD_MFMA_PATCHES) {
        PatchPlan pp{};
        pp.eligible = true;
        pp.npx = p->patch.npx; pp.npy = p->patch.npy; pp.nseg = p->patch.nseg; pp.segl = p->patch.segl;
        pp.ntasks = p->patch.ntasks; pp.lds_bytes = p->patch.lds_bytes; pp.pby = p->patch.pby; pp.f32acc = p->patch.f32acc; pp.planar = p->patch.planar;
        double advantage = 0.85 * 1.15 * std::pow(p->is_complex ? 1.45 : 1.2, (double)std::max(p->M - 4, 0)) * (p->patch.f32acc ? 1.3 : 1.0);
        if (p->spread_method_req == NUFFT_SPREAD_MFMA_PATCHES) advantage = 0.0;
        const int slots = p->wave_slots;
        const int clo = -((p->M + 2) / 4), chi = (3 + p->M) / 4;
        const size_t ncols = (size_t)pp.npx * pp.npy;
        NUFFT_HIP(launch_patch_tasks(s.g, pp, clo, chi, p->d_offsets, np, slots, advantage, p->d_patch_choice, p->bal.d_slots, p->d_patch_cols,
                                     p->d_patch_cols + ncols, static_cast<uint2*>(p->d_patch_tasks), stream));
    }
    if (p->spread_method == NUFFT_SPREAD_MARCHING_RING) {
        const double adv_env = option_double("NUFFT_SMARCH_ADVANTAGE", 0.0);
        double advantage = p->smarch.halo == 2 ? 0.93 * 1.4 : 0.85 * 1.3;
        if (adv_env > 0.0) advantage = adv_env;
        if (p->spread_method_req == NUFFT_SPREAD_MARCHING_RING) advantage = 0.0;
        const size_t ncols = (size_t)p->smarch.ct.ncolx * p->smarch.ct.ncoly;
        NUFFT_HIP(launch_smarch_tasks(s.g, p->smarch, p->d_offsets, np, std::max(1, p->num_cus / (p->C * p->smarch.parts)), advantage, p->d_smarch_choice, p->bal.d_slots, p->d_smarch_cols,
                                      p->d_smarch_cols + ncols, static_cast<uint2*>(p->d_smarch_tasks), stream));
    }
    if (p->interp_march) {
        const double rho = (double)np / (double)std::max<int64_t>(p->grid_elems, 1), mr = (double)p->M / 4.0;
        const double fitted = (rho + 0.038 * std::pow(mr, 1.85)) / (1.09 * rho + 0.0086 * std::pow(mr, 1.2));
        const double advantage = p->interp_march_mode == 2 ? 0.0 : fitted;
        const double rho_star = (0.038 * std::pow(mr, 1.85) - 0.0086 * std::pow(mr, 1.2)) / 0.09;
        const size_t ncols = (size_t)p->march_ct.ncolx * p->march_ct.ncoly;
        NUFFT_HIP(launch_march_tasks(s.g, p->march_ct, p->d_offsets, np, p->num_cus, advantage, 2.5 * rho_star, p->d_march_choice, p->d_march_cols,
                                     p->d_march_cols + ncols, static_cast<uint2*>(p->d_march_tasks), stream));
    }
    if (coarse) {
        NUFFT_HIP(launch_binsort_coarse_finish(s, stream));
        if ((rc = balance())) return rc;
    } else if (p->sort_feedback && p->coarse.enabled && !p->dense_now) {
        NUFFT_HIP(launch_sort_feedback(p->coarse.flag_a, p->coarse.flag_b, p->sort_feedback, ++p->sort_seq, stream));
    }
    if (p->debug_tasks) {
        auto check = [&](const char* name, const ColumnTasks& ct, const void* tab, const uint32_t* choice) {
            const size_t ncols = (size_t)ct.ncolx * ct.ncoly, ntab = (size_t)column_task_table_entries(ct, p->tile.nb[2]);
            std::vector<uint32_t> h(2 * ntab), ch(8);
            (void)hipStreamSynchronize(stream);
            (void)hipMemcpy(h.data(), tab, ntab * 8, hipMemcpyDeviceToHost);
            (void)hipMemcpy(ch.data(), choice, 32, hipMemcpyDeviceToHost);
            std::vector<std::vector<std::pair<int, int>>> segs(ncols);
            size_t used = 0, maxlen = 0;
            for (size_t t = 0; t < ntab; ++t) {
                const uint32_t c = h[2 * t], y = h[2 * t + 1];
                if (!y) continue;
                ++used;
                if (c >= ncols) { fprintf(stderr, "[tasks %s] entry %zu: column %u out of range\n", name, t, c); continue; }
                segs[c].push_back({(int)(y & 0xffffu), (int)(y >> 16)});
                maxlen = std::max(maxlen, (size_t)((y >> 16) - (y & 0xffffu)));
            }
            size_t bad = 0;
            for (size_t c = 0; c < ncols; ++c) {
                std::sort(segs[c].begin(), segs[c].end());
                int z = 0;
                for (auto& sg : segs[c]) { if (sg.first != z) ++bad; z = sg.second; }
                if (z != p->tile.nb[2]) ++bad;
            }
            fprintf(stderr, "[tasks %s] columns %zu, table %zu, in use %zu, longest %zu layers, flag %u, uniform %u, bad columns %zu\n", name, ncols, ntab,
                    used, maxlen, ch[2], ch[3], bad);
        };
        if (p->spread_method == NUFFT_SPREAD_MFMA_PATCHES) {
            ColumnTasks ct{p->patch.npx, p->patch.npy, 4, p->patch.pby, p->patch.nseg, p->patch.segl, p->patch.ntasks, 1, 0, 0, 0};
            check("patches", ct, p->d_patch_tasks, p->d_patch_choice);
        }
        if (p->interp_march) check("ring", p->march_ct, p->d_march_tasks, p->d_march_choice);
        if (p->spread_method == NUFFT_SPREAD_MARCHING_RING) check("spreading ring", p->smarch.ct, p->d_smarch_tasks, p->d_smarch_choice);
    }
    p->Np = np;
    p->counts_clean = np > 0;
    return NUFFT_OK;
}

int nufft_spread_engine_used(nufft_plan* p, int* engine_out, void* stream_) {
    int rc = require_points(p);
    if (rc) return rc;
    if (!engine_out) return fail(NUFFT_ERR_INVALID_ARG, "null output");
    *engine_out = NUFFT_SPREAD_LDS_TILES;
    if (p->spread_method != NUFFT_SPREAD_MFMA_PATCHES && p->spread_method != NUFFT_SPREAD_MARCHING_RING) return NUFFT_OK;
    DeviceGuard guard(p->device);
    hipStream_t stream = static_cast<hipStream_t>(stream_);
    uint32_t flag = 0;
    const uint32_t* src = p->spread_method == NUFFT_SPREAD_MFMA_PATCHES ? p->d_patch_choice : p->d_smarch_choice;
    NUFFT_HIP(hipMemcpyAsync(&flag, src + 2, sizeof(flag), hipMemcpyDeviceToHost, stream));
    NUFFT_HIP(hipStreamSynchronize(stream));
    *engine_out = flag ? p->spread_method : NUFFT_SPREAD_LDS_TILES;
    if (flag && p->spread_method == NUFFT_SPREAD_MARCHING_RING && p->dense_now) *engine_out = NUFFT_SPREAD_MARCHING_RING_DENSE;
    return NUFFT_OK;
}

int nufft_sort_columns_used(nufft_plan* p, int* used_out, void* stream_) {
    int rc = require_points(p);
    if (rc) return rc;
    if (!used_out) return fail(NUFFT_ERR_INVALID_ARG, "null output");
    *used_out = 0;
    if (!p->coarse.enabled && !p->slab.enabled) return NUFFT_OK;
    DeviceGuard guard(p->device);
    hipStream_t stream = static_cast<hipStream_t>(stream_);
    uint32_t fa = 0, fb = 0;
    if (p->slab.enabled && !p->coarse_now) {
        NUFFT_HIP(hipMemcpyAsync(&fa, p->slab.flag_a, sizeof(fa), hipMemcpyDeviceToHost, stream));
        NUFFT_HIP(hipStreamSynchronize(stream));
        *used_out = fa != 0 ? 2 : 0;
        return NUFFT_OK;
    }
    NUFFT_HIP(hipMemcpyAsync(&fa, p->coarse.flag_a, sizeof(fa), hipMemcpyDeviceToHost, stream));
    NUFFT_HIP(hipMemcpyAsync(&fb, p->coarse.flag_b, sizeof(fb), hipMemcpyDeviceToHost, stream));
    NUFFT_HIP(hipStreamSynchronize(stream));
    *used_out = (fa != 0 && fb != 0) ? 1 : 0;
    return NUFFT_OK;
}

int nufft_interp_engine_used(nufft_plan* p, int* engine_out, void* stream_) {
    int rc = require_points(p);
    if (rc) return rc;
    if (!engine_out) return fail(NUFFT_ERR_INVALID_ARG, "null output");
    *engine_out = NUFFT_INTERP_LDS_TILES;
    if (!p->interp_march) return NUFFT_OK;
    DeviceGuard guard(p->device);
    hipStream_t stream = static_cast<hipStream_t>(stream_);
    uint32_t flag = 0;
    NUFFT_HIP(hipMemcpyAsync(&flag, p->d_march_choice + 2, sizeof(flag), hipMemcpyDeviceToHost, stream));
    NUFFT_HIP(hipStreamSynchronize(stream));
    if (flag) *engine_out = NUFFT_INTERP_MARCHING_RING;
    return NUFFT_OK;
}

int64_t nufft_sizeof_params(void) { return (int64_t)sizeof(nufft_params); }
int64_t nufft_sizeof_info(void) { return (int64_t)sizeof(nufft_info); }

int nufft_fill_zeros(nufft_plan* p, void* stream_) {
    int rc = require_device(p);
    if (rc) return rc;
    DeviceGuard guard(p->device);
    hipStream_t stream = static_cast<hipStream_t>(stream_);
    StageTimer tm(p, NUFFT_STAGE_T1_ZERO, stream);
    note_capture(p, stream);
    if ((rc = void_halo(p, stream))) return rc;
    NUFFT_HIP(launch_zero_fill(p->d_us, (size_t)p->grid_elems * value_bytes(p) * p->C, stream));
    return NUFFT_OK;
}

static int spread_impl(nufft_plan* p, const void* const* values_in, void* stream_, bool defer_halo) {
    int rc = require_points(p);
    if (rc) return rc;
    if (!values_in) return fail(NUFFT_ERR_INVALID_ARG, "null value table");
    for (int c = 0; c < p->C; ++c)
        if (p->Np > 0 && !values_in[c]) return fail(NUFFT_ERR_INVALID_ARG, "null value vector");
    DeviceGuard guard(p->device);
    hipStream_t stream = static_cast<hipStream_t>(stream_);
    StageTimer tm(p, NUFFT_STAGE_T1_SPREAD, stream);
    note_capture(p, stream);
    TileKernelArgs a = tile_args(p, false);
    a.values_in = values_in;
    if (p->balance_enabled)
        NUFFT_HIP(launch_zero_split_tiles(p->dtype, a.g, p->D, p->is_complex, p->C, p->bal.d_nslices, p->d_us,
                                          p->grid_elems * (p->is_complex ? 2 : 1), stream));
    NUFFT_HIP(launch_spread(a, stream));
    if (p->spread_method == NUFFT_SPREAD_MARCHING_RING) {
        NUFFT_HIP(launch_spread_march(a, p->smarch, p->d_smarch_choice + 2, static_cast<const uint2*>(p->d_smarch_tasks), p->d_smarch_choice + kHaloStateWord, p->dense_now, stream));
        if (halo_plan(p)) {
            p->halo_hint = true;
            if (!defer_halo && (rc = complete_halo(p, stream))) return rc;
        }
    }
    if (p->spread_method == NUFFT_SPREAD_MFMA_PATCHES) {
        const uint32_t* enabled = p->d_patch_choice + 2;
        const int64_t vstride = p->Np * (p->is_complex ? 2 : 1);
        if (p->patch.planar)
            NUFFT_HIP(launch_gather_planar(p->dtype, p->D, p->d_sorted, p->Np, values_in, p->C, p->cb_point_weights, p->d_vsorted, enabled, stream));
        else
            for (int c = 0; c < p->C; ++c)
                NUFFT_HIP(launch_gather_values(p->dtype, p->is_complex, p->D, p->d_sorted, p->Np, values_in[c], p->cb_point_weights,
                                               static_cast<char*>(p->d_vsorted) + (size_t)c * vstride * real_bytes(p), enabled, stream));
        PatchPlan pp{};
        pp.eligible = true;
        pp.npx = p->patch.npx; pp.npy = p->patch.npy; pp.nseg = p->patch.nseg; pp.segl = p->patch.segl;
        pp.ntasks = p->patch.ntasks; pp.lds_bytes = p->patch.lds_bytes; pp.pby = p->patch.pby; pp.f32acc = p->patch.f32acc; pp.planar = p->patch.planar;
        NUFFT_HIP(launch_spread_patch(a, pp, p->d_vsorted, vstride, enabled, static_cast<const uint2*>(p->d_patch_tasks), stream));
    }
    return NUFFT_OK;
}

// ... 184 lines not shown

int nufft_exec_type1(nufft_plan* p, void* const* uhat_out, const void* const* values_in, void* stream) {
    int rc = require_points(p);
    if (rc) return rc;
    if (!uhat_out || !values_in) return fail(NUFFT_ERR_INVALID_ARG, "null argument");
    if ((rc = nufft_spread_deferred(p, values_in, stream))) return rc;
    if ((rc = nufft_fft_forward(p, stream))) return rc;
    return nufft_deconvolve_truncate(p, uhat_out, stream);
}

namespace {
struct CallbackScope {
    nufft_plan* p;
    CallbackScope(nufft_plan* plan, const nufft_callbacks* cb) : p(plan) {
        p->cb_point_weights = cb ? cb->point_weights : nullptr;
        p->cb_mode_factors = cb ? cb->mode_factors : nullptr;
    }
    ~CallbackScope() { p->cb_point_weights = p->cb_sticky_weights; p->cb_mode_factors = p->cb_sticky_factors; }
};
}

int nufft_set_callbacks(nufft_plan* p, const nufft_callbacks* cb) {
    if (!p) return fail(NUFFT_ERR_INVALID_ARG, "null plan");
    p->cb_sticky_weights = p->cb_point_weights = cb ? cb->point_weights : nullptr;
    p->cb_sticky_factors = p->cb_mode_factors = cb ? cb->mode_factors : nullptr;
    return NUFFT_OK;
}

int nufft_exec_type1_cb(nufft_plan* p, void* const* uhat_out, const void* const* values_in, const nufft_callbacks* cb,
                        void* stream) {
    if (!p) return fail(NUFFT_ERR_INVALID_ARG, "null plan");
    CallbackScope scope(p, cb);
    return nufft_exec_type1(p, uhat_out, values_in, stream);
}

int nufft_exec_type2_cb(nufft_plan* p, void* const* values_out, const void* const* uhat_in, const nufft_callbacks* cb,
                        void* stream) {
    if (!p) return fail(NUFFT_ERR_INVALID_ARG, "null plan");
    CallbackScope scope(p, cb);
    return nufft_exec_type2(p, values_out, uhat_in, stream);
}

int nufft_exec_type2(nufft_plan* p, void* const* values_out, const void* const* uhat_in, void* stream) {
    int rc = require_points(p);
    if (rc) return rc;
    if (!values_out || !uhat_in) return fail(NUFFT_ERR_INVALID_ARG, "null argument");
    if ((rc = nufft_deconvolve_pad(p, uhat_in, stream))) return rc;
    if ((rc = nufft_fft_backward(p, stream))) return rc;
    return nufft_interpolate(p, values_out, stream);
}

int nufft_grid_ptr(const nufft_plan* p, int which, int component, void** out_ptr, int64_t* out_bytes) {
    int rc = require_device(p);
    if (rc) return rc;
    if (!out_ptr || component < 0 || component >= p->C) return fail(NUFFT_ERR_INVALID_ARG, "bad argument");
    if (which == 0) {
        if (halo_maybe_pending(p))
            return fail(NUFFT_ERR_INVALID_ARG, "us lacks the side buffer of a deferred spread (nufft_spread_deferred / nufft_exec_type1 on a "
                                               "ring_halo plan): call nufft_complete_grid first, or use nufft_copy_grid");
        const size_t bytes = (size_t)p->grid_elems * value_bytes(p);
        *out_ptr = static_cast<char*>(p->d_us) + bytes * component;
        if (out_bytes) *out_bytes = (int64_t)bytes;
    } else if (which == 1 && !p->is_complex) {
        const size_t bytes = (size_t)p->pspec_elems * 2 * real_bytes(p);
        *out_ptr = static_cast<char*>(p->d_uhat) + bytes * component;
        if (out_bytes) *out_bytes = (int64_t)bytes;
    } else {
        return fail(NUFFT_ERR_INVALID_ARG, "which must be 0 (us) or 1 (ûs, real plans only)");
    }
    return NUFFT_OK;
}

int nufft_complete_grid(nufft_plan* p, void* stream_) {
    int rc = require_device(p);
    if (rc) return rc;
    DeviceGuard guard(p->device);
    note_capture(p, static_cast<hipStream_t>(stream_));
    return complete_halo(p, static_cast<hipStream_t>(stream_));
}

int nufft_copy_grid(nufft_plan* p, int which, int component, void* dst, int64_t capacity_bytes, void* stream_) {
    int rc = require_device(p);
    if (rc) return rc;
    if (component < 0 || component >= p->C) return fail(NUFFT_ERR_INVALID_ARG, "bad argument");
    if (which != 0 && !(which == 1 && !p->is_complex)) return fail(NUFFT_ERR_INVALID_ARG, "which must be 0 (us) or 1 (ûs, real plans only)");
    if (!dst) return fail(NUFFT_ERR_INVALID_ARG, "null destination");
    const size_t bytes = which == 0 ? (size_t)p->grid_elems * value_bytes(p) : (size_t)p->pspec_elems * 2 * real_bytes(p);
    if (capacity_bytes < (int64_t)bytes) return fail(NUFFT_ERR_DIM_MISMATCH, "destination buffer too small");
    DeviceGuard guard(p->device);
    hipStream_t stream = static_cast<hipStream_t>(stream_);
    if (which == 0) {
        note_capture(p, stream);
        if ((rc = complete_halo(p, stream))) return rc;
    }
    const char* src = static_cast<const char*>(which == 0 ? p->d_us : p->d_uhat) + bytes * (size_t)component;
    NUFFT_HIP(hipMemcpyAsync(dst, src, bytes, hipMemcpyDeviceToDevice, stream));
    return NUFFT_OK;
}

int nufft_get_sort_result(nufft_plan* p, int32_t* perm_host, int64_t perm_capacity, uint32_t* tile_offsets_host,
                          int64_t offsets_capacity, void* stream_) {
    int rc = require_points(p);
    if (rc) return rc;
    DeviceGuard guard(p->device);
    hipStream_t stream = static_cast<hipStream_t>(stream_);
    if (perm_host) {
        if (perm_capacity < p->Np) return fail(NUFFT_ERR_DIM_MISMATCH, "perm buffer too small");
        if (p->Np > 0) {
            int32_t* tmp = nullptr;
            NUFFT_HIP(hipMalloc(reinterpret_cast<void**>(&tmp), (size_t)p->Np * sizeof(int32_t)));
            hipError_t e = launch_extract_perm(p->dtype, p->D, p->d_sorted, p->Np, tmp, stream);
            if (e == hipSuccess) e = hipMemcpyAsync(perm_host, tmp, (size_t)p->Np * sizeof(int32_t), hipMemcpyDeviceToHost, stream);
            if (e == hipSuccess) e = hipStreamSynchronize(stream);
            (void)hipFree(tmp);
            NUFFT_HIP(e);
        }
    }
    if (tile_offsets_host) {
        const int64_t n = p->tile.nbins + 1;
        if (offsets_capacity < n) return fail(NUFFT_ERR_DIM_MISMATCH, "offset buffer too small");
        NUFFT_HIP(hipMemcpyAsync(tile_offsets_host, p->d_offsets, (size_t)n * sizeof(uint32_t), hipMemcpyDeviceToHost, stream));
        NUFFT_HIP(hipStreamSynchronize(stream));
    }
    return NUFFT_OK;
}

int nufft_set_timing(nufft_plan* p, int enable) {
    int rc = require_device(p);
    if (rc) return rc;
    p->timing = enable != 0;
    if (!p->timing)
        for (int s = 0; s < NUFFT_NUM_STAGES; ++s) p->ev_valid[s] = false;
    return NUFFT_OK;
}

int nufft_get_stage_times(nufft_plan* p, float* ms_out) {
    int rc = require_device(p);
    if (rc) return rc;
    if (!ms_out) return fail(NUFFT_ERR_INVALID_ARG, "null output");
    DeviceGuard guard(p->device);
    for (int s = 0; s < NUFFT_NUM_STAGES; ++s) {
        ms_out[s] = -1.0f;
        if (!p->ev_valid[s]) continue;
        hipEvent_t a = static_cast<hipEvent_t>(p->ev_begin[s]);
        hipEvent_t b = static_cast<hipEvent_t>(p->ev_end[s]);
        NUFFT_HIP(hipEventSynchronize(b));
        float ms = 0.f;
        NUFFT_HIP(hipEventElapsedTime(&ms, a, b));
        ms_out[s] = ms;
    }
    return NUFFT_OK;
}

}
```

Measured before the change: 3.078 billion.

## Chain set_points coarse sort, task planning and balance into fewer fused kernels

Adds a short-chain path, on by default through NUFFT_SETPOINTS_CHAIN, for the coarse sort in set_points. It collects the ring and march column-task work into RingTasks and runs a fused coarse-plan launch plus a short balance, which merges tile work, sums, scan and descriptor fill. Existing kernels are refactored into device bodies so fused kernels can reuse them, with agent-scope coherent loads and ticket counters replacing kernel boundaries. The goal is to cut the many small launches and serial dependencies in set_points, at the cost of more complex cross-block synchronisation and extra allocations.

```diff
diff --git a/nonuniformffts.jl_amd/csrc/balance.hip b/nonuniformffts.jl_amd/csrc/balance.hip
--- a/nonuniformffts.jl_amd/csrc/balance.hip
+++ b/nonuniformffts.jl_amd/csrc/balance.hip
@@ -4,6 +4,8 @@
 #include <atomic>
 #include <hipcub/hipcub.hpp>
 
+#include "block_scan.h"
+#include "fill_desc.h"
 #include "device_common.h"
 #include "kernels.h"
 
@@ -11,13 +13,9 @@
 
 constexpr int kWorkLanes = 16;
 
-__global__ __launch_bounds__(256) void tile_work_kernel(Geom g, int D, int M, const uint32_t* __restrict__ offsets,
-                                                       uint32_t* __restrict__ work, const uint32_t* skip_a, const uint32_t* skip_b) {
-    if (skip_a && *skip_a != 0u && *skip_b != 0u) return;
+__device__ __forceinline__ uint32_t tile_work_of(const Geom& g, int D, int M, const uint32_t* __restrict__ offsets, int wave, int lane) {
     const int nsp = g.sp.ntiles, nip = g.ip.ntiles;
-    const int wave = (blockIdx.x * blockDim.x + threadIdx.x) / kWorkLanes;
-    const int lane = threadIdx.x & (kWorkLanes - 1);
-    if (wave >= nsp + nip) return;
+    if (wave >= nsp + nip) return 0u;
     const bool interp = wave >= nsp;
     const TileShape& ts = interp ? g.ip : g.sp;
     int rem = interp ? wave - nsp : wave, t[3];
@@ -48,7 +46,15 @@
         sum += offsets[bin0 + (sg ? seg[0].len[1] : seg[0].len[0])] - offsets[bin0];
     }
     for (int o = kWorkLanes / 2; o > 0; o >>= 1) sum += __shfl_down(sum, o, kWorkLanes);
-    if (lane == 0) work[wave] = sum;
+    return sum;
+}
+__global__ __launch_bounds__(256) void tile_work_kernel(Geom g, int D, int M, const uint32_t* __restrict__ offsets,
+                                                       uint32_t* __restrict__ work, const uint32_t* skip_a, const uint32_t* skip_b) {
+    if (skip_a && *skip_a != 0u && *skip_b != 0u) return;
+    const int wave = (blockIdx.x * blockDim.x + threadIdx.x) / kWorkLanes;
+    const int lane = threadIdx.x & (kWorkLanes - 1);
+    const uint32_t sum = tile_work_of(g, D, M, offsets, wave, lane);
+    if (lane == 0 && wave < g.sp.ntiles + g.ip.ntiles) work[wave] = sum;
 }
 
 constexpr int kSumBlocks = 128;
@@ -107,23 +113,7 @@
                                                        uint32_t ip_base, uint2* __restrict__ desc,
                                                        uint32_t* __restrict__ slots_in_use, const uint32_t* skip_a, const uint32_t* skip_b,
                                                        const uint32_t* sp_served) {
-    constexpr int kLanes = 8;
-    const int t = (blockIdx.x * blockDim.x + threadIdx.x) / kLanes, lane = threadIdx.x & (kLanes - 1);
-    if (skip_a && *skip_a != 0u && *skip_b != 0u) {
-        if (blockIdx.x == 0 && threadIdx.x < 2) slots_in_use[threadIdx.x] = 0u;
-        return;
-    }
-    if (t >= nsp + nip) return;
-    const uint32_t split = desc_off[nsp];
-    const bool interp = t >= nsp;
-    const uint32_t S = nslices[t];
-    const uint32_t off = interp ? ip_base + (desc_off[t] - split) : desc_off[t];
-    const uint32_t tile = interp ? (uint32_t)(t - nsp) : (uint32_t)t;
-    for (uint32_t s = lane; s < S; s += kLanes) desc[off + s] = make_uint2(tile, (s << 16) | S);
-    if (t == 0 && lane == 0) {
-        slots_in_use[0] = (sp_served && *sp_served != 0u) ? 0u : split;
-        slots_in_use[1] = desc_off[nsp + nip] - split;
-    }
+    fill_desc_body(nslices, desc_off, nsp, nip, ip_base, desc, slots_in_use, skip_a, skip_b, sp_served, (int)blockIdx.x);
 }
 
 size_t balance_work_words(int ntiles_both) {
@@ -155,11 +145,12 @@
 
 constexpr int kPatchMaxLayers = 2048;
 
-__global__ __launch_bounds__(256) void patch_column_sums_kernel(Geom g, int npx, int npy, int pbx, int pby, int segl, const uint32_t* __restrict__ offsets,
-                                                               uint32_t* __restrict__ colsum, uint32_t* __restrict__ choice) {
+template <typename Off>
+__device__ __forceinline__ void column_sums_body(const Geom& g, int npx, int npy, int pbx, int pby, int segl, const Off& offsets,
+                                                 uint32_t* __restrict__ colsum, uint32_t* __restrict__ choice, int blk) {
     __shared__ uint32_t seg_all[256 / kWave][kPatchMaxLayers];
     const int w = threadIdx.x / kWave, lane = threadIdx.x & (kWave - 1);
-    const int c = blockIdx.x * (256 / kWave) + w;
+    const int c = blk * (256 / kWave) + w;
     if (c >= npx * npy) return;
     const int bx0 = (c % npx) * pbx, by0 = (c / npx) * pby;
     const int ncx = min(pbx, g.nb[0] - bx0), ncy = min(pby, g.nb[1] - by0);
@@ -189,20 +180,25 @@
         atomicMax(&choice[6], heaviest);
     }
 }
-
-__global__ __launch_bounds__(1024) void patch_task_counts_kernel(int ncols, int ntasks, int ntab, int nseg, int min_seg, int max_seg, unsigned long long np,
-                                                                unsigned long long limit, unsigned long long slots_eff, int uniform_always,
-                                                                const uint32_t* __restrict__ colsum, uint32_t* __restrict__ first,
-                                                                uint2* __restrict__ tasktab, uint32_t* __restrict__ choice,
-                                                                uint32_t* __restrict__ slots_in_use) {
-    __shared__ uint32_t part[1024];
+__global__ __launch_bounds__(256) void patch_column_sums_kernel(Geom g, int npx, int npy, int pbx, int pby, int segl, const uint32_t* __restrict__ offsets,
+                                                               uint32_t* __restrict__ colsum, uint32_t* __restrict__ choice) {
+    column_sums_body(g, npx, npy, pbx, pby, segl, offsets, colsum, choice, (int)blockIdx.x);
+}
+
+template <int NT, bool COH>
+__device__ __forceinline__ void task_counts_body(int ncols, int ntasks, int ntab, int nseg, int min_seg, int max_seg, unsigned long long np,
+                                                 unsigned long long limit, unsigned long long slots_eff, int uniform_always,
+                                                 const uint32_t* __restrict__ colsum, uint32_t* __restrict__ first,
+                                                 uint2* __restrict__ tasktab, uint32_t* __restrict__ choice,
+                                                 uint32_t* __restrict__ slots_in_use) {
+    __shared__ uint32_t part[NT];
     __shared__ uint32_t carry;
     __shared__ int uniform_mode;
     const int tid = threadIdx.x;
     if (tid == 0) {
         carry = 0;
         const double mean = (double)np / (double)ntasks;
-        const uint32_t heaviest = choice[6];
+        const uint32_t heaviest = COH ? ld_agent(choice + 6) : choice[6];
         choice[6] = 0u;
         choice[kHaloStateWord] = 0u;
         uniform_mode = (double)heaviest <= 1.1 * mean + 5.0 * sqrt(mean) + 8.0;
@@ -215,19 +211,19 @@
     }
     __syncthreads();
     const bool uni = uniform_mode != 0;
-    for (int c0 = 0; c0 < ncols; c0 += 1024) {
+    for (int c0 = 0; c0 < ncols; c0 += NT) {
         const int c = c0 + tid;
         uint32_t S = 0;
         if (c < ncols) {
             if (uni) S = (uint32_t)nseg;
             else {
-                S = np ? (uint32_t)(((unsigned long long)ntasks * colsum[c] + np / 2) / np) : 1u;
+                S = np ? (uint32_t)(((unsigned long long)ntasks * (COH ? ld_agent(colsum + c) : colsum[c]) + np / 2) / np) : 1u;
                 S = S < (uint32_t)min_seg ? (uint32_t)min_seg : (S > (uint32_t)max_seg ? (uint32_t)max_seg : S);
             }
         }
         part[tid] = S;
         __syncthreads();
-        for (int o = 1; o < 1024; o <<= 1) {
+        for (int o = 1; o < NT; o <<= 1) {
             const uint32_t v = tid >= o ? part[tid - o] : 0u;
             __syncthreads();
             part[tid] += v;
@@ -235,23 +231,30 @@
         }
         if (c < ncols) first[c] = carry + part[tid] - S;
         __syncthreads();
-        if (tid == 1023) carry += part[1023];
+        if (tid == NT - 1) carry += part[NT - 1];
         __syncthreads();
     }
     if (tid == 0) first[ncols] = carry;
-    for (int t = (int)carry + tid; t < ntab; t += 1024) tasktab[t] = make_uint2(0u, 0u);
-}
-
-__global__ __launch_bounds__(256) void patch_split_kernel(Geom g, int npx, int npy, int pbx, int pby, int clo, int chi, int zq, int segl, int maxlen,
-                                                         const uint32_t* __restrict__ offsets, const uint32_t* __restrict__ first,
-                                                         unsigned long long limit, unsigned long long limit_cut, unsigned long long slots_eff, int uniform_always,
-                                                         double rho_eff_max, unsigned long long np,
-                                                         uint2* __restrict__ tasktab, uint32_t* __restrict__ choice,
-                                                         uint32_t* __restrict__ slots_in_use) {
+    for (int t = (int)carry + tid; t < ntab; t += NT) tasktab[t] = make_uint2(0u, 0u);
+}
+__global__ __launch_bounds__(1024) void patch_task_counts_kernel(int ncols, int ntasks, int ntab, int nseg, int min_seg, int max_seg, unsigned long long np,
+                                                                unsigned long long limit, unsigned long long slots_eff, int uniform_always,
+                                                                const uint32_t* __restrict__ colsum, uint32_t* __restrict__ first,
+                                                                uint2* __restrict__ tasktab, uint32_t* __restrict__ choice,
+                                                                uint32_t* __restrict__ slots_in_use) {
+    task_counts_body<1024, false>(ncols, ntasks, ntab, nseg, min_seg, max_seg, np, limit, slots_eff, uniform_always, colsum, first, tasktab, choice, slots_in_use);
+}
+
+__device__ __forceinline__ bool column_split_body(const Geom& g, int npx, int npy, int pbx, int pby, int clo, int chi, int zq, int segl, int maxlen,
+                                                  const uint32_t* __restrict__ offsets, const uint32_t* __restrict__ first,
+                                                  unsigned long long limit, unsigned long long limit_cut, unsigned long long slots_eff, int uniform_always,
+                                                  double rho_eff_max, unsigned long long np,
+                                                  uint2* __restrict__ tasktab, uint32_t* __restrict__ choice,
+                                                  uint32_t* __restrict__ slots_in_use, int blk, int nblk) {
     __shared__ uint32_t cum_all[256 / kWave][kPatchMaxLayers + 1];
     __shared__ uint16_t bnd_all[256 / kWave][kPatchMaxLayers + 2];
     const int w = threadIdx.x / kWave, lane = threadIdx.x & (kWave - 1);
-    const int c = blockIdx.x * (256 / kWave) + w;
+    const int c = blk * (256 / kWave) + w;
     const int nz = g.nb[2];
     if (choice[3] != 0u) {
         if (c < npx * npy) {
@@ -261,7 +264,7 @@
                 tasktab[k * (uint32_t)(npx * npy) + (uint32_t)c] = make_uint2((uint32_t)c, z1 > z0 ? ((uint32_t)z1 << 16) | (uint32_t)z0 : 0u);
             }
         }
-        return;
+        return false;
     }
     uint32_t* cum = cum_all[w];
     unsigned long long wsum = 0, wsq = 0;
@@ -346,11 +349,13 @@
             atomicAdd(reinterpret_cast<unsigned long long*>(choice + 8), wsq);
         }
     }
+    __shared__ uint32_t split_last;
     __syncthreads();
     if (threadIdx.x == 0) {
         __threadfence();
         const uint32_t ticket = atomicAdd(&choice[1], 1u);
-        if (ticket == gridDim.x - 1) {
+        split_last = ticket == (uint32_t)nblk - 1u ? 1u : 0u;
+        if (ticket == (uint32_t)nblk - 1u) {
             __threadfence();
             const unsigned long long mx = atomicExch(&choice[0], 0u);
             const unsigned long long sum = atomicExch(reinterpret_cast<unsigned long long*>(choice + 4), 0ull);
@@ -366,20 +371,34 @@
             if (patches && slots_in_use) slots_in_use[0] = 0u;
         }
     }
+    __syncthreads();
+    return split_last != 0u;
+}
+__global__ __launch_bounds__(256) void patch_split_kernel(Geom g, int npx, int npy, int pbx, int pby, int clo, int chi, int zq, int segl, int maxlen,
+                                                         const uint32_t* __restrict__ offsets, const uint32_t* __restrict__ first,
+                                                         unsigned long long limit, unsigned long long limit_cut, unsigned long long slots_eff, int uniform_always,
+                                                         double rho_eff_max, unsigned long long np,
+                                                         uint2* __restrict__ tasktab, uint32_t* __restrict__ choice,
+                                                         uint32_t* __restrict__ slots_in_use) {
+    column_split_body(g, npx, npy, pbx, pby, clo, chi, zq, segl, maxlen, offsets, first, limit, limit_cut, slots_eff, uniform_always, rho_eff_max, np, tasktab,
+                      choice, slots_in_use, (int)blockIdx.x, (int)gridDim.x);
 }
 
 constexpr int kPatchSortMax = 16384;
 
-__global__ __launch_bounds__(1024) void patch_task_sort_kernel(int ntasks, int npad, const uint32_t* __restrict__ first, int ncols,
-                                                              const uint32_t* __restrict__ choice, uint2* __restrict__ tasktab) {
-    extern __shared__ __attribute__((aligned(16))) unsigned char smem_sort[];
-    unsigned long long* key = reinterpret_cast<unsigned long long*>(smem_sort);
+template <int NT, bool COH>
+__device__ __forceinline__ void task_sort_body(int ntasks, int npad, const uint32_t* __restrict__ first, int ncols,
+                                               const uint32_t* __restrict__ choice, uint2* __restrict__ tasktab, unsigned long long* key) {
     const int tid = threadIdx.x;
     if (choice[3] != 0u) return;
-    for (int t = tid; t < npad; t += 1024) {
+    for (int t = tid; t < npad; t += NT) {
         unsigned long long k = ~0ull;
         if (t < ntasks) {
-            const uint2 e = tasktab[t];
+            uint2 e;
+            if (COH) {
+                const unsigned long long raw = __hip_atomic_load(reinterpret_cast<const unsigned long long*>(tasktab + t), __ATOMIC_RELAXED, __HIP_MEMORY_SCOPE_AGENT);
+                e = make_uint2((uint32_t)raw, (uint32_t)(raw >> 32));
+            } else e = tasktab[t];
             if (e.y != 0u) k = ((unsigned long long)(t - first[e.x]) << 48) | ((unsigned long long)e.x << 32) | e.y;
         }
         key[t] = k;
@@ -387,7 +406,7 @@
     __syncthreads();
     for (int size = 2; size <= npad; size <<= 1) {
         for (int stride = size >> 1; stride > 0; stride >>= 1) {
-            for (int i = tid; i < npad / 2; i += 1024) {
+            for (int i = tid; i < npad / 2; i += NT) {
                 const int lo = 2 * i - (i & (stride - 1));
                 const int hi = lo + stride;
                 const bool up = (lo & size) == 0;
@@ -397,24 +416,49 @@
             __syncthreads();
         }
     }
-    for (int t = tid; t < ntasks; t += 1024) {
+    for (int t = tid; t < ntasks; t += NT) {
         const unsigned long long k = key[t];
         tasktab[t] = k == ~0ull ? make_uint2(0u, 0u) : make_uint2((uint32_t)(k >> 32) & 0xffffu, (uint32_t)k);
     }
 }
+__global__ __launch_bounds__(1024) void patch_task_sort_kernel(int ntasks, int npad, const uint32_t* __restrict__ first, int ncols,
+                                                              const uint32_t* __restrict__ choice, uint2* __restrict__ tasktab) {
+    extern __shared__ __attribute__((aligned(16))) unsigned char smem_sort[];
+    task_sort_body<1024, false>(ntasks, npad, first, ncols, choice, tasktab, reinterpret_cast<unsigned long long*>(smem_sort));
+}
+
+constexpr int kSplitSortMax = 8192;
+__global__ void column_split2_kernel(Geom g, const uint32_t* __restrict__ offsets, RingTasks ra, RingTasks rb, unsigned long long np, int sort_here);
+__global__ void task_sort2_kernel(RingTasks ra, RingTasks rb);
 
 bool patch_tasks_supported(const Geom& g) { return g.nb[2] <= kPatchMaxLayers; }
 
 hipError_t prepare_column_tasks() {
-    return hipFuncSetAttribute(reinterpret_cast<const void*>(patch_task_sort_kernel), hipFuncAttributeMaxDynamicSharedMemorySize, kPatchSortMax * 8);
+    hipError_t e = hipFuncSetAttribute(reinterpret_cast<const void*>(patch_task_sort_kernel), hipFuncAttributeMaxDynamicSharedMemorySize, kPatchSortMax * 8);
+    if (e == hipSuccess) e = hipFuncSetAttribute(reinterpret_cast<const void*>(task_sort2_kernel), hipFuncAttributeMaxDynamicSharedMemorySize, kPatchSortMax * 8);
+    if (e == hipSuccess) e = hipFuncSetAttribute(reinterpret_cast<const void*>(column_split2_kernel), hipFuncAttributeMaxDynamicSharedMemorySize, kSplitSortMax * 8);
+    return e;
 }
 int patch_task_table_entries(const PatchPlan& pp) { return pp.ntasks + 2 * pp.npx * pp.npy; }
 
 static hipError_t launch_column_tasks(const Geom& g, const ColumnTasks& ct, const uint32_t* offsets, int64_t np, unsigned long long limit,
                                       unsigned long long limit_cut, unsigned long long slots_eff, bool uniform_always, uint32_t* choice, uint32_t* slots_in_use,
-                                      uint32_t* colsum, uint32_t* first, uint2* tasktab, hipStream_t stream, double rho_eff_max = 0.0) {
+                                      uint32_t* colsum, uint32_t* first, uint2* tasktab, hipStream_t stream, double rho_eff_max = 0.0,
+                                      RingTasks* collect = nullptr) {
     const int ncols = ct.ncolx * ct.ncoly, wpb = 256 / kWave;
     const int ntab = column_task_table_entries(ct, g.nb[2]);
+    if (collect) {
+        RingTasks& r = *collect;
+        r.ct = ct; r.ncols = ncols; r.ntab = ntab; r.nblocks = (ncols + wpb - 1) / wpb;
+        r.min_seg = ct.maxlen > 0 ? (g.nb[2] + ct.maxlen - 1) / ct.maxlen : 1;
+        r.max_seg = g.nb[2] / ct.zq;
+        r.npad = 0;
+        if (ntab <= kPatchSortMax && ncols < 65536) for (r.npad = 2; r.npad < ntab;) r.npad <<= 1;
+        r.uniform_always = uniform_always ? 1 : 0;
+        r.limit = limit; r.limit_cut = limit_cut; r.slots_eff = slots_eff; r.rho_eff_max = rho_eff_max;
+        r.choice = choice; r.slots_in_use = slots_in_use; r.colsum = colsum; r.first = first; r.tasktab = tasktab;
+        return hipSuccess;
+    }
     hipLaunchKernelGGL(patch_column_sums_kernel, dim3((unsigned)((ncols + wpb - 1) / wpb)), dim3(256), 0, stream, g, ct.ncolx, ct.ncoly, ct.bxw, ct.byw,
                        ct.segl, offsets, colsum, choice);
     const int min_seg = ct.maxlen > 0 ? (g.nb[2] + ct.maxlen - 1) / ct.maxlen : 1;
@@ -443,23 +487,154 @@
 }
 
 hipError_t launch_march_tasks(const Geom& g, const ColumnTasks& ct, const uint32_t* offsets, int64_t np, int cus, double advantage, double rho_eff_max,
-                              uint32_t* choice, uint32_t* colsum, uint32_t* first, uint2* tasktab, hipStream_t stream) {
+                              uint32_t* choice, uint32_t* colsum, uint32_t* first, uint2* tasktab, hipStream_t stream, RingTasks* collect) {
     const unsigned long long slots_eff = (unsigned long long)std::max(1, std::min(cus, ct.ntasks));
     const bool always = advantage <= 0.0;
     const unsigned long long limit = always ? ~0ull / (slots_eff + 1ull) : (unsigned long long)(advantage * (double)np / (double)cus) + 64ull;
     const unsigned long long limit_cut = always ? limit : (unsigned long long)(0.85 * advantage * (double)np / (double)cus) + 64ull;
     return launch_column_tasks(g, ct, offsets, np, limit, limit_cut, slots_eff, always, choice, nullptr, colsum, first, tasktab, stream,
-                               always ? 0.0 : rho_eff_max);
+                               always ? 0.0 : rho_eff_max, collect);
 }
 
 hipError_t launch_smarch_tasks(const Geom& g, const SMarchPlan& sp, const uint32_t* offsets, int64_t np, int cus, double advantage,
-                               uint32_t* choice, uint32_t* slots_in_use, uint32_t* colsum, uint32_t* first, uint2* tasktab, hipStream_t stream) {
+                               uint32_t* choice, uint32_t* slots_in_use, uint32_t* colsum, uint32_t* first, uint2* tasktab, hipStream_t stream,
+                               RingTasks* collect) {
     const ColumnTasks& ct = sp.ct;
     const unsigned long long slots_eff = (unsigned long long)std::max(1, std::min(cus, ct.ntasks));
     const double infl0 = (double)(ct.segl + sp.hlo + sp.hhi) / (double)ct.segl;
     const unsigned long long limit = advantage > 0.0 ? (unsigned long long)(advantage * infl0 * (double)np / (double)cus) + 64ull
                                                      : ~0ull / (slots_eff + 1ull);
-    return launch_column_tasks(g, ct, offsets, np, limit, limit, slots_eff, advantage <= 0.0, choice, slots_in_use, colsum, first, tasktab, stream);
+    return launch_column_tasks(g, ct, offsets, np, limit, limit, slots_eff, advantage <= 0.0, choice, slots_in_use, colsum, first, tasktab, stream, 0.0, collect);
+}
+
+constexpr int kMaxKeyGroups = (kCoarseMaxKeys + kCoarseKeyGroup - 1) / kCoarseKeyGroup;
+struct KeyOffsetsDev {
+    const uint32_t* within;
+    const uint32_t* gbase;
+    uint32_t nb0, nb1, cbx, cby, ncx, ncy;
+    __device__ __forceinline__ uint32_t operator[](int64_t b64) const {
+        const uint32_t b = (uint32_t)b64;
+        const uint32_t bx = b % nb0, t = b / nb0, by = t % nb1, bz = t / nb1;
+        const uint32_t k = (bz * ncy + (by + cby - 1u) / cby) * ncx + (by % cby == 0u ? (bx + cbx - 1u) / cbx : 0u);
+        return gbase[k / kCoarseKeyGroup] + within[k];
+    }
+};
+
+__global__ __launch_bounds__(kScanThreads) void coarse_plan_kernel(Geom g, KeyOffsets ko, uint32_t* __restrict__ offsets, int fill_blocks, RingTasks ra, RingTasks rb,
+                                                                  unsigned long long np, uint32_t* ticket) {
+    __shared__ __attribute__((aligned(16))) uint32_t gbase[kMaxKeyGroups + 8];
+    block_exclusive_scan((int64_t)ko.ngroups + 1, gbase, [&](int64_t i) {
+        uint4 v;
+        v.x = i < ko.ngroups ? ko.grouptot[i] : 0u;
+        v.y = i + 1 < ko.ngroups ? ko.grouptot[i + 1] : 0u;
+        v.z = i + 2 < ko.ngroups ? ko.grouptot[i + 2] : 0u;
+        v.w = i + 3 < ko.ngroups ? ko.grouptot[i + 3] : 0u;
+        return v;
+    });
+    __syncthreads();
+    const KeyOffsetsDev kd{ko.within, gbase, (uint32_t)ko.nb0, (uint32_t)ko.nb1, (uint32_t)ko.cbx, (uint32_t)ko.cby, (uint32_t)ko.ncx, (uint32_t)ko.ncy};
+    const int b = (int)blockIdx.x;
+    if (b < fill_blocks) {
+        const int64_t n = (int64_t)g.nbins + 1;
+        for (int64_t i = (int64_t)b * kScanThreads + threadIdx.x; i < n; i += (int64_t)fill_blocks * kScanThreads) offsets[i] = kd[i];
+        return;
+    }
+    const bool second = b - fill_blocks >= ra.nblocks;
+    const RingTasks& r = second ? rb : ra;
+    column_sums_body(g, r.ct.ncolx, r.ct.ncoly, r.ct.bxw, r.ct.byw, r.ct.segl, kd, r.colsum, r.choice, b - fill_blocks - (second ? ra.nblocks : 0));
+    if (!last_workgroup(ticket, (uint32_t)(ra.nblocks + rb.nblocks))) return;
+    task_counts_body<kScanThreads, true>(ra.ncols, ra.ct.ntasks, ra.ntab, ra.ct.nseg, ra.min_seg, ra.max_seg, np, ra.limit, ra.slots_eff, ra.uniform_always, ra.colsum,
+                                         ra.first, ra.tasktab, ra.choice, ra.slots_in_use);
+    __syncthreads();
+    task_counts_body<kScanThreads, true>(rb.ncols, rb.ct.ntasks, rb.ntab, rb.ct.nseg, rb.min_seg, rb.max_seg, np, rb.limit, rb.slots_eff, rb.uniform_always, rb.colsum,
+                                         rb.first, rb.tasktab, rb.choice, rb.slots_in_use);
+}
+
+__global__ __launch_bounds__(256) void column_split2_kernel(Geom g, const uint32_t* __restrict__ offsets, RingTasks ra, RingTasks rb, unsigned long long np,
+                                                            int sort_here) {
+    extern __shared__ __attribute__((aligned(16))) unsigned char smem_split2[];
+    const bool second = (int)blockIdx.x >= ra.nblocks;
+    const RingTasks& r = second ? rb : ra;
+    const bool last = column_split_body(g, r.ct.ncolx, r.ct.ncoly, r.ct.bxw, r.ct.byw, r.ct.clo, r.ct.chi, r.ct.zq, r.ct.segl, r.ct.maxlen, offsets, r.first, r.limit, r.limit_cut,
+                      r.slots_eff, r.uniform_always, r.rho_eff_max, np, r.tasktab, r.choice, r.slots_in_use, (int)blockIdx.x - (second ? ra.nblocks : 0), r.nblocks);
+    if (last && sort_here && r.npad) task_sort_body<256, true>(r.ntab, r.npad, r.first, r.ncols, r.choice, r.tasktab, reinterpret_cast<unsigned long long*>(smem_split2));
+}
+
+__global__ __launch_bounds__(1024) void task_sort2_kernel(RingTasks ra, RingTasks rb) {
+    extern __shared__ __attribute__((aligned(16))) unsigned char smem_sort2[];
+    const RingTasks& r = blockIdx.x ? rb : ra;
+    if (r.npad == 0) return;
+    task_sort_body<1024, false>(r.ntab, r.npad, r.first, r.ncols, r.choice, r.tasktab, reinterpret_cast<unsigned long long*>(smem_sort2));
+}
+
+hipError_t launch_coarse_plan(const Geom& g, const CoarseSort& cs, uint32_t* offsets, int64_t np, const RingTasks& ra, const RingTasks& rb, hipStream_t stream) {
+    const int ngroups = coarse_key_groups(cs.nkeys);
+    KeyOffsets ko{cs.keyoff, cs.keyoff + ngroups * kCoarseKeyGroup + 4, ngroups, g.nb[0], g.nb[1], cs.cbx, cs.cby, cs.ncx, cs.ncy};
+    const int fill_blocks = (int)std::min<int64_t>(512, ((int64_t)g.nbins + 1 + 4 * kScanThreads - 1) / (4 * kScanThreads));
+    hipLaunchKernelGGL(coarse_plan_kernel, dim3((unsigned)(fill_blocks + ra.nblocks + rb.nblocks)), dim3(kScanThreads), 0, stream, g, ko, offsets, fill_blocks, ra, rb,
+                       (unsigned long long)np, cs.tickets + kTicketTaskCounts);
+    const int npad = std::max(ra.npad, rb.npad);
+    const bool sort_here = npad <= kSplitSortMax;
+    hipLaunchKernelGGL(column_split2_kernel, dim3((unsigned)(ra.nblocks + rb.nblocks)), dim3(256), sort_here ? (size_t)npad * 8 : 0, stream, g, offsets, ra, rb,
+                       (unsigned long long)np, sort_here ? 1 : 0);
+    if (npad && !sort_here)
+        hipLaunchKernelGGL(task_sort2_kernel, dim3(2), dim3(1024), (size_t)std::max(ra.npad, rb.npad) * 8, stream, ra, rb);
+    return hipGetLastError();
+}
+
+__global__ __launch_bounds__(kScanThreads) void balance_work_scan_kernel(Geom g, int D, int M, const uint32_t* __restrict__ offsets, uint32_t* __restrict__ work,
+                                                                        uint32_t extra_sp, uint32_t extra_ip, uint32_t smax, uint32_t* __restrict__ nslices,
+                                                                        uint32_t* __restrict__ desc_off, unsigned long long* __restrict__ totals,
+                                                                        const uint32_t* skip_a, const uint32_t* skip_b, uint32_t* ticket) {
+    __shared__ unsigned long long tot[2];
+    const int nsp = g.sp.ntiles, nip = g.ip.ntiles, n = nsp + nip;
+    const int tid = threadIdx.x;
+    if (*skip_a != 0u && *skip_b != 0u) {
+        for (int t = blockIdx.x * kScanThreads + tid; t <= n; t += gridDim.x * kScanThreads) {
+            if (t < n) nslices[t] = 1u;
+            desc_off[t] = (uint32_t)t;
+        }
+        return;
+    }
+    if (tid < 2) tot[tid] = 0ull;
+    __syncthreads();
+    const int tile = (blockIdx.x * kScanThreads + tid) / kWorkLanes;
+    const uint32_t sum = tile_work_of(g, D, M, offsets, tile, tid & (kWorkLanes - 1));
+    if ((tid & (kWorkLanes - 1)) == 0 && tile < n) {
+        work[tile] = sum;
+        if (sum) atomicAdd(&tot[tile >= nsp ? 1 : 0], (unsigned long long)sum);
+    }
+    __syncthreads();
+    if (tid < 2 && tot[tid]) atomicAdd(&totals[tid], tot[tid]);
+    if (!last_workgroup(ticket, gridDim.x)) return;
+    if (tid < 2) tot[tid] = atomicExch(&totals[tid], 0ull);
+    __syncthreads();
+    const unsigned long long W0 = tot[0], W1 = tot[1];
+    auto slices_of = [&](int64_t t) -> uint32_t {
+        if (t >= n) return 0u;
+        const bool interp = t >= nsp;
+        const unsigned long long W = interp ? W1 : W0;
+        unsigned long long s = W ? (unsigned long long)ld_agent(work + t) * (interp ? extra_ip : extra_sp) / W : 0ull;
+        if (s > smax - 1) s = smax - 1;
+        return 1u + (uint32_t)s;
+    };
+    block_exclusive_scan((int64_t)n + 1, desc_off, [&](int64_t i) {
+        uint4 v;
+        v.x = slices_of(i); v.y = slices_of(i + 1); v.z = slices_of(i + 2); v.w = slices_of(i + 3);
+        if (i <= n) nslices[i] = v.x;
+        if (i + 1 <= n) nslices[i + 1] = v.y;
+        if (i + 2 <= n) nslices[i + 2] = v.z;
+        if (i + 3 <= n) nslices[i + 3] = v.w;
+        return v;
+    });
+}
+
+hipError_t launch_balance_short(const BalanceArgs& b, unsigned long long* totals, uint32_t* ticket, hipStream_t stream) {
+    const int nsp = b.g.sp.ntiles, nip = b.g.ip.ntiles, n = nsp + nip;
+    const int tiles_per_block = kScanThreads / kWorkLanes;
+    hipLaunchKernelGGL(balance_work_scan_kernel, dim3((unsigned)((n + tiles_per_block - 1) / tiles_per_block)), dim3(kScanThreads), 0, stream, b.g, b.D, b.M, b.offsets,
+                       b.work, b.enabled ? b.extra_sp : 0u, b.enabled ? b.extra_ip : 0u, b.smax, b.nslices, b.desc_off, totals, b.skip_a, b.skip_b, ticket);
+    return hipGetLastError();
 }
 
 template <typename T>
diff --git a/nonuniformffts.jl_amd/csrc/binsort.hip b/nonuniformffts.jl_amd/csrc/binsort.hip
--- a/nonuniformffts.jl_amd/csrc/binsort.hip
+++ b/nonuniformffts.jl_amd/csrc/binsort.hip
@@ -1,6 +1,8 @@
 #include <hip/hip_runtime.h>
 #include <hipcub/hipcub.hpp>
 
+#include "block_scan.h"
+#include "fill_desc.h"
 #include "device_common.h"
 #include "kernels.h"
 
@@ -32,12 +34,11 @@
 constexpr int kCountPPT = 4;
 constexpr int kCountSlots = 2048;
 constexpr uint32_t kEmptyKey = 0xFFFFFFFFu;
+static_assert(kCountThreads == kScanThreads, "fine_count_scan_kernel scans with the workgroup that counts");
 
 template <typename T, int D>
-__global__ __launch_bounds__(kCountThreads) void bin_count_kernel(BinArgs<T, D> a, uint32_t* __restrict__ counts,
-                                                                 uint2* __restrict__ binrank, const uint32_t* skip_a, const uint32_t* skip_b) {
+__device__ __forceinline__ void bin_count_body(const BinArgs<T, D>& a, uint32_t* __restrict__ counts, uint2* __restrict__ binrank) {
     __shared__ uint32_t keys[kCountSlots], cnt[kCountSlots], base[kCountSlots];
-    if (skip_a && *skip_a != 0u && *skip_b != 0u) return;
     constexpr int kChunkPts = kCountThreads * kCountPPT;
     const int tid = threadIdx.x;
     const int64_t nchunks = (a.np + kChunkPts - 1) / kChunkPts;
@@ -75,26 +76,37 @@
         __syncthreads();
     }
 }
-
+template <typename T, int D>
+__global__ __launch_bounds__(kCountThreads) void bin_count_kernel(BinArgs<T, D> a, uint32_t* __restrict__ counts,
+                                                                 uint2* __restrict__ binrank, const uint32_t* skip_a, const uint32_t* skip_b) {
+    if (skip_a && *skip_a != 0u && *skip_b != 0u) return;
+    bin_count_body<T, D>(a, counts, binrank);
+}
+
+template <typename T, int D>
+__device__ __forceinline__ void bin_scatter_body(const BinArgs<T, D>& a, const uint32_t* __restrict__ offsets, const uint2* __restrict__ binrank,
+                                                 PointRec<T, D>* __restrict__ sorted, uint32_t* __restrict__ counts, int ncounts, int blk, int nblk) {
+    const int64_t stride = (int64_t)nblk * 256;
+    for (int64_t i = (int64_t)blk * 256 + threadIdx.x; i < ncounts; i += stride) counts[i] = 0u;
+    for (int64_t p = (int64_t)blk * 256 + threadIdx.x; p < a.np; p += stride) {
+        const uint2 br = binrank[p];
+        PointRec<T, D> rec;
+#pragma unroll
+        for (int d = 0; d < D; ++d) {
+            const T xf = transform_and_fold(a.x[d][p], a.point_transform);
+            rec.r[d] = to_grid_units(xf, a.g.Nover[d]);
+        }
+        rec.idx = (int32_t)p;
+        sorted[offsets[br.x] + br.y] = rec;
+    }
+}
 template <typename T, int D>
 __global__ __launch_bounds__(256) void bin_scatter_kernel(BinArgs<T, D> a, const uint32_t* __restrict__ offsets,
                                                          const uint2* __restrict__ binrank,
                                                          PointRec<T, D>* __restrict__ sorted, uint32_t* __restrict__ counts, int ncounts,
                                                          const uint32_t* skip_a, const uint32_t* skip_b) {
     if (skip_a && *skip_a != 0u && *skip_b != 0u) return;
-    const int64_t stride = (int64_t)gridDim.x * blockDim.x;
-    for (int64_t i = (int64_t)blockIdx.x * blockDim.x + threadIdx.x; i < ncounts; i += stride) counts[i] = 0u;
-    for (int64_t p = (int64_t)blockIdx.x * blockDim.x + threadIdx.x; p < a.np; p += stride) {
-        const uint2 br = binrank[p];
-        PointRec<T, D> rec;
-#pragma unroll
-        for (int d = 0; d < D; ++d) {
-            const T xf = transform_and_fold(a.x[d][p], a.point_transform);
-            rec.r[d] = to_grid_units(xf, a.g.Nover[d]);
-        }
-        rec.idx = (int32_t)p;
-        sorted[offsets[br.x] + br.y] = rec;
-    }
+    bin_scatter_body<T, D>(a, offsets, binrank, sorted, counts, ncounts, (int)blockIdx.x, (int)gridDim.x);
 }
 
 __global__ void zero_fill_kernel(uint4* __restrict__ dst, int64_t n16, uint32_t* __restrict__ tail, int ntail) {
@@ -490,6 +502,136 @@
     return hipGetLastError();
 }
 
+
+__global__ __launch_bounds__(256) void coarse_prefix_keys_kernel(CoarseGeom c, int groups, uint32_t* __restrict__ table, uint32_t* __restrict__ within,
+                                                                uint32_t* __restrict__ grouptot) {
+    __shared__ uint32_t part[4][kCoarseKeyGroup];
+    const int lane = threadIdx.x & 63, q = threadIdx.x >> 6;
+    const int k = blockIdx.x * kCoarseKeyGroup + lane;
+    const int per = (groups + 3) / 4, w0 = min(q * per, groups), w1 = min(w0 + per, groups);
+    uint32_t sum = 0u;
+    if (k < c.nkeys) {
+        int w = w0;
+        for (; w + 8 <= w1; w += 8) {
+            uint32_t v[8];
+#pragma unroll
+            for (int u = 0; u < 8; ++u) v[u] = table[(size_t)(w + u) * c.nkeys + k];
+#pragma unroll
+            for (int u = 0; u < 8; ++u) sum += v[u];
+        }
+        for (; w < w1; ++w) sum += table[(size_t)w * c.nkeys + k];
+    }
+    part[q][lane] = sum;
+    __syncthreads();
+    uint32_t run = 0u, total = 0u;
+#pragma unroll
+    for (int j = 0; j < 4; ++j) {
+        const uint32_t t = part[j][lane];
+        if (j < q) run += t;
+        total += t;
+    }
+    if (k < c.nkeys) {
+        int w = w0;
+        for (; w + 8 <= w1; w += 8) {
+            uint32_t v[8];
+#pragma unroll
+            for (int u = 0; u < 8; ++u) v[u] = table[(size_t)(w + u) * c.nkeys + k];
+#pragma unroll
+            for (int u = 0; u < 8; ++u) {
+                table[(size_t)(w + u) * c.nkeys + k] = run;
+                run += v[u];
+            }
+        }
+        for (; w < w1; ++w) {
+            const uint32_t v = table[(size_t)w * c.nkeys + k];
+            table[(size_t)w * c.nkeys + k] = run;
+            run += v;
+        }
+    }
+    if (q == 0) {
+        uint32_t incl = total;
+#pragma unroll
+        for (int o = 1; o < 64; o <<= 1) {
+            const uint32_t t = (uint32_t)__shfl_up((int)incl, o);
+            if (lane >= o) incl += t;
+        }
+        within[k] = incl - total;
+        if (lane == 63) grouptot[blockIdx.x] = incl;
+    }
+}
+
+template <typename T>
+__global__ __launch_bounds__(kCountThreads) void fine_count_scan_kernel(BinArgs<T, 3> a, uint32_t* __restrict__ counts, uint2* __restrict__ binrank,
+                                                                       uint32_t* __restrict__ offsets, const uint32_t* fa, const uint32_t* fb, uint32_t* ticket) {
+    if (*fa != 0u && *fb != 0u) return;
+    bin_count_body<T, 3>(a, counts, binrank);
+    if (!last_workgroup(ticket, gridDim.x)) return;
+    const int64_t n = (int64_t)a.g.nbins + 1;
+    block_exclusive_scan(n, offsets, [&](int64_t i) {
+        if (i + 3 < n) return *reinterpret_cast<const uint4*>(counts + i);
+        uint4 v;
+        v.x = ld_agent(counts + i);
+        v.y = i + 1 < n ? ld_agent(counts + i + 1) : 0u;
+        v.z = i + 2 < n ? ld_agent(counts + i + 2) : 0u;
+        v.w = 0u;
+        return v;
+    });
+}
+
+template <typename T>
+__global__ __launch_bounds__(256) void fine_scatter_desc_kernel(BinArgs<T, 3> a, const uint32_t* __restrict__ offsets, const uint2* __restrict__ binrank,
+                                                               PointRec<T, 3>* __restrict__ sorted, uint32_t* __restrict__ counts, int ncounts, int ndesc,
+                                                               const uint32_t* __restrict__ nslices, const uint32_t* __restrict__ desc_off, int nsp, int nip,
+                                                               uint32_t ip_base, uint2* __restrict__ desc, uint32_t* __restrict__ slots_in_use,
+                                                               const uint32_t* fa, const uint32_t* fb, const uint32_t* sp_served) {
+    const int blk = (int)blockIdx.x;
+    if (blk < ndesc) {
+        fill_desc_body(nslices, desc_off, nsp, nip, ip_base, desc, slots_in_use, fa, fb, sp_served, blk);
+        return;
+    }
+    if (*fa != 0u && *fb != 0u) return;
+    bin_scatter_body<T, 3>(a, offsets, binrank, sorted, counts, ncounts, blk - ndesc, (int)gridDim.x - ndesc);
+}
+
+template <typename T>
+static hipError_t coarse_count_short_t(const SortArgs& s, hipStream_t stream) {
+    const CoarseGeom c = coarse_geom(s.cs);
+    if (!s.counts_clean) {
+        hipError_t e = launch_zero_fill(s.counts, sizeof(uint32_t) * (size_t)(s.g.nbins + 1), stream);
+        if (e != hipSuccess) return e;
+    }
+    hipLaunchKernelGGL((coarse_count_kernel<T>), dim3((unsigned)s.cs.groups), dim3(kCoarseThreads), (size_t)c.nkeys * 4, stream, bin_args3<T>(s), c, s.cs.table);
+    const int ngroups = coarse_key_groups(c.nkeys);
+    hipLaunchKernelGGL(coarse_prefix_keys_kernel, dim3((unsigned)ngroups), dim3(256), 0, stream, c, s.cs.groups, s.cs.table, s.cs.keyoff,
+                       s.cs.keyoff + ngroups * kCoarseKeyGroup + 4);
+    return hipGetLastError();
+}
+
+template <typename T>
+static hipError_t coarse_finish_short_t(const SortArgs& s, const BalanceArgs& q, hipStream_t stream) {
+    const CoarseGeom c = coarse_geom(s.cs);
+    const BinArgs<T, 3> a = bin_args3<T>(s);
+    const uint32_t *fa = s.cs.flag_a, *fb = s.cs.flag_b;
+    if (s.np > 0) {
+        int64_t blocks = (s.np + kCountThreads * kCountPPT - 1) / (kCountThreads * kCountPPT);
+        if (blocks > 256 * 16) blocks = 256 * 16;
+        hipLaunchKernelGGL((fine_count_scan_kernel<T>), dim3((unsigned)blocks), dim3(kCountThreads), 0, stream, a, s.counts, static_cast<uint2*>(s.binrank),
+                           s.offsets, fa, fb, s.cs.tickets + kTicketFineCount);
+    }
+    hipLaunchKernelGGL((coarse_scatter_kernel<T>), dim3((unsigned)s.cs.groups), dim3(kCoarseThreads), (size_t)c.nkeys * 4, stream, a, c, s.cs.table, s.offsets,
+                       static_cast<PointRec<T, 3>*>(s.sorted), s.counts, fa, fb, s.cs.fb_a, s.cs.fb_b,
+                       (s.cs.fb_a && s.cs.fb_b) ? s.cs.feedback : (uint32_t*)nullptr, s.cs.seq);
+    hipError_t e = launch_balance_short(q, reinterpret_cast<unsigned long long*>(s.cs.tickets + kTicketWorkTotals), s.cs.tickets + kTicketBalance, stream);
+    if (e != hipSuccess) return e;
+    const int nsp = q.g.sp.ntiles, nip = q.g.ip.ntiles, ndesc = (nsp + nip + 31) / 32;
+    int64_t blocks = (s.np + 255) / 256;
+    if (blocks > 256 * 32) blocks = 256 * 32;
+    hipLaunchKernelGGL((fine_scatter_desc_kernel<T>), dim3((unsigned)(ndesc + blocks)), dim3(256), 0, stream, a, s.offsets, static_cast<const uint2*>(s.binrank),
+                       static_cast<PointRec<T, 3>*>(s.sorted), s.counts, s.g.nbins + 1, ndesc, q.nslices, q.desc_off, nsp, nip, (uint32_t)nsp + q.extra_sp, q.desc,
+                       q.slots_in_use, fa, fb, q.sp_served);
+    return hipGetLastError();
+}
+
 __global__ void sort_feedback_kernel(const uint32_t* ra, const uint32_t* rb, uint32_t* feedback, uint32_t seq) {
     __atomic_store_n(&feedback[0], *ra, __ATOMIC_RELAXED);
     __atomic_store_n(&feedback[1], *rb, __ATOMIC_RELAXED);
@@ -502,7 +644,11 @@
 }
 
 hipError_t launch_binsort_coarse_count(const SortArgs& s, hipStream_t stream) {
+    if (s.cs.chain) return s.dtype == NUFFT_F32 ? coarse_count_short_t<float>(s, stream) : coarse_count_short_t<double>(s, stream);
     return s.dtype == NUFFT_F32 ? coarse_count_t<float>(s, stream) : coarse_count_t<double>(s, stream);
+}
+hipError_t launch_binsort_coarse_finish_short(const SortArgs& s, const BalanceArgs& q, hipStream_t stream) {
+    return s.dtype == NUFFT_F32 ? coarse_finish_short_t<float>(s, q, stream) : coarse_finish_short_t<double>(s, q, stream);
 }
 hipError_t launch_binsort_coarse_finish(const SortArgs& s, hipStream_t stream) {
     return s.dtype == NUFFT_F32 ? coarse_finish_t<float>(s, stream) : coarse_finish_t<double>(s, stream);
diff --git a/nonuniformffts.jl_amd/csrc/block_scan.h b/nonuniformffts.jl_amd/csrc/block_scan.h
--- /dev/null
+++ b/nonuniformffts.jl_amd/csrc/block_scan.h
@@ -0,0 +1,86 @@
+#pragma once
+
+#include <hip/hip_runtime.h>
+#include <cstdint>
+
+namespace nufft {
+
+constexpr int kScanThreads = 256;
+constexpr int kScanSteps = 8;
+
+__device__ __forceinline__ uint32_t ld_agent(const uint32_t* p) { return __hip_atomic_load(p, __ATOMIC_RELAXED, __HIP_MEMORY_SCOPE_AGENT); }
+
+__device__ __forceinline__ bool last_workgroup(uint32_t* ticket, uint32_t nblocks) {
+    __shared__ uint32_t is_last;
+    __syncthreads();
+    if (threadIdx.x == 0) {
+        __threadfence();
+        const uint32_t t = atomicAdd(ticket, 1u);
+        is_last = t == nblocks - 1u ? 1u : 0u;
+        if (is_last) {
+            __threadfence();
+            atomicExch(ticket, 0u);
+        }
+    }
+    __syncthreads();
+    return is_last != 0u;
+}
+
+template <typename Load4>
+__device__ __forceinline__ uint32_t block_exclusive_scan(int64_t n, uint32_t* __restrict__ out, Load4 load4) {
+    __shared__ uint32_t wsum[2][kScanSteps][kScanThreads / 64];
+    const int tid = threadIdx.x, lane = tid & 63, wave = tid >> 6;
+    constexpr int64_t kRound = (int64_t)kScanSteps * kScanThreads * 4;
+    uint32_t carry = 0u;
+    int par = 0;
+    for (int64_t base = 0; base < n; base += kRound, par ^= 1) {
+        uint4 v[kScanSteps];
+        uint32_t incl[kScanSteps], tsum[kScanSteps];
+#pragma unroll
+        for (int s = 0; s < kScanSteps; ++s) {
+            const int64_t i = base + ((int64_t)s * kScanThreads + tid) * 4;
+            v[s] = i < n ? load4(i) : make_uint4(0u, 0u, 0u, 0u);
+        }
+#pragma unroll
+        for (int s = 0; s < kScanSteps; ++s) {
+            tsum[s] = v[s].x + v[s].y + v[s].z + v[s].w;
+            uint32_t x = tsum[s];
+#pragma unroll
+            for (int o = 1; o < 64; o <<= 1) {
+                const uint32_t t = (uint32_t)__shfl_up((int)x, o);
+                if (lane >= o) x += t;
+            }
+            incl[s] = x;
+            if (lane == 63) wsum[par][s][wave] = x;
+        }
+        __syncthreads();
+        uint32_t before = carry;
+#pragma unroll
+        for (int s = 0; s < kScanSteps; ++s) {
+            uint32_t b = before;
+#pragma unroll
+            for (int w = 0; w < kScanThreads / 64; ++w) {
+                const uint32_t t = wsum[par][s][w];
+                if (w < wave) b += t;
+                before += t;
+            }
+            uint32_t run = b + incl[s] - tsum[s];
+            const int64_t i = base + ((int64_t)s * kScanThreads + tid) * 4;
+            if (i + 3 < n) {
+                uint4 o4;
+                o4.x = run; run += v[s].x;
+                o4.y = run; run += v[s].y;
+                o4.z = run; run += v[s].z;
+                o4.w = run;
+                *reinterpret_cast<uint4*>(out + i) = o4;
+            } else if (i < n) {
+                const uint32_t e[4] = {v[s].x, v[s].y, v[s].z, v[s].w};
+                for (int j = 0; j < 4 && i + j < n; ++j) { out[i + j] = run; run += e[j]; }
+            }
+        }
+        carry = before;
+    }
+    return carry;
+}
+
+}
diff --git a/nonuniformffts.jl_amd/csrc/column_tasks.h b/nonuniformffts.jl_amd/csrc/column_tasks.h
--- a/nonuniformffts.jl_amd/csrc/column_tasks.h
+++ b/nonuniformffts.jl_amd/csrc/column_tasks.h
@@ -69,7 +69,14 @@
     const uint32_t* fb_b;
     uint32_t* feedback;
     uint32_t seq;
+    int chain;
+    uint32_t* keyoff;
+    uint32_t* tickets;
 };
+constexpr int kTicketFineCount = 1, kTicketTaskCounts = 2, kTicketBalance = 3, kTicketWorkTotals = 4;
+constexpr int kCoarseKeyGroup = 64;
+inline int coarse_key_groups(int nkeys) { return (nkeys + kCoarseKeyGroup - 1) / kCoarseKeyGroup; }
+inline int coarse_keyoff_words(int nkeys) { return coarse_key_groups(nkeys) * kCoarseKeyGroup + 4 + ((coarse_key_groups(nkeys) + 4 + 3) & ~3); }
 constexpr int kSlabMaxBins = 4096;
 constexpr int kHaloStateWord = 12;
 constexpr int kSlabOverfill = 8;
diff --git a/nonuniformffts.jl_amd/csrc/fill_desc.h b/nonuniformffts.jl_amd/csrc/fill_desc.h
--- /dev/null
+++ b/nonuniformffts.jl_amd/csrc/fill_desc.h
@@ -0,0 +1,32 @@
+#pragma once
+
+#include <hip/hip_runtime.h>
+#include <cstdint>
+
+namespace nufft {
+
+__device__ __forceinline__ void fill_desc_body(const uint32_t* __restrict__ nslices,
+                                                       const uint32_t* __restrict__ desc_off, int nsp, int nip,
+                                                       uint32_t ip_base, uint2* __restrict__ desc,
+                                                       uint32_t* __restrict__ slots_in_use, const uint32_t* skip_a, const uint32_t* skip_b,
+                                                       const uint32_t* sp_served, int blk) {
+    constexpr int kLanes = 8;
+    const int t = (blk * 256 + (int)threadIdx.x) / kLanes, lane = threadIdx.x & (kLanes - 1);
+    if (skip_a && *skip_a != 0u && *skip_b != 0u) {
+        if (blk == 0 && threadIdx.x < 2) slots_in_use[threadIdx.x] = 0u;
+        return;
+    }
+    if (t >= nsp + nip) return;
+    const uint32_t split = desc_off[nsp];
+    const bool interp = t >= nsp;
+    const uint32_t S = nslices[t];
+    const uint32_t off = interp ? ip_base + (desc_off[t] - split) : desc_off[t];
+    const uint32_t tile = interp ? (uint32_t)(t - nsp) : (uint32_t)t;
+    for (uint32_t s = lane; s < S; s += kLanes) desc[off + s] = make_uint2(tile, (s << 16) | S);
+    if (t == 0 && lane == 0) {
+        slots_in_use[0] = (sp_served && *sp_served != 0u) ? 0u : split;
+        slots_in_use[1] = desc_off[nsp + nip] - split;
+    }
+}
+
+}
diff --git a/nonuniformffts.jl_amd/csrc/kernels.h b/nonuniformffts.jl_amd/csrc/kernels.h
--- a/nonuniformffts.jl_amd/csrc/kernels.h
+++ b/nonuniformffts.jl_amd/csrc/kernels.h
@@ -34,9 +34,27 @@
 hipError_t prepare_binsort_slab(int dtype, int lds_bytes);
 hipError_t launch_binsort_coarse_count(const SortArgs& s, hipStream_t stream);
 hipError_t launch_binsort_coarse_finish(const SortArgs& s, hipStream_t stream);
+struct BalanceArgs;
+hipError_t launch_binsort_coarse_finish_short(const SortArgs& s, const BalanceArgs& q, hipStream_t stream);
 hipError_t launch_sort_feedback(const uint32_t* ra, const uint32_t* rb, uint32_t* feedback, uint32_t seq, hipStream_t stream);
 hipError_t launch_zero_fill(void* dst, size_t bytes, hipStream_t stream);
 hipError_t launch_extract_perm(int dtype, int D, const void* sorted, int64_t np, int32_t* perm_dev, hipStream_t stream);
+
+struct KeyOffsets {
+    const uint32_t* within;
+    const uint32_t* grouptot;
+    int ngroups;
+    int nb0, nb1, cbx, cby, ncx, ncy;
+};
+struct RingTasks {
+    ColumnTasks ct;
+    int ncols, ntab, nblocks, min_seg, max_seg, npad, uniform_always;
+    unsigned long long limit, limit_cut, slots_eff;
+    double rho_eff_max;
+    uint32_t *choice, *slots_in_use, *colsum, *first;
+    uint2* tasktab;
+};
+hipError_t launch_coarse_plan(const Geom& g, const CoarseSort& cs, uint32_t* offsets, int64_t np, const RingTasks& a, const RingTasks& b, hipStream_t stream);
 
 struct BalanceArgs {
     Geom g;
@@ -59,6 +77,7 @@
 size_t balance_scan_tmp_bytes(int ntiles_both);
 size_t balance_work_words(int ntiles_both);
 hipError_t launch_balance(const BalanceArgs& b, hipStream_t stream);
+hipError_t launch_balance_short(const BalanceArgs& b, unsigned long long* totals, uint32_t* ticket, hipStream_t stream);
 hipError_t launch_zero_split_tiles(int dtype, const Geom& g, int D, int is_complex, int C, const uint32_t* nslices,
                                    void* grid, int64_t grid_stride_reals, hipStream_t stream);
 
@@ -121,7 +140,7 @@
 };
 PatchPlan patch_plan(int dtype, int is_complex, int D, int M, const Geom& g, bool other, bool allow_f32acc = true, int planar_nc = 0);
 hipError_t launch_march_tasks(const Geom& g, const ColumnTasks& ct, const uint32_t* offsets, int64_t np, int cus, double advantage, double rho_eff_max,
-                              uint32_t* choice, uint32_t* colsum, uint32_t* first, uint2* tasktab, hipStream_t stream);
+                              uint32_t* choice, uint32_t* colsum, uint32_t* first, uint2* tasktab, hipStream_t stream, RingTasks* collect = nullptr);
 hipError_t launch_patch_tasks(const Geom& g, const PatchPlan& pp, int clo, int chi, const uint32_t* offsets, int64_t np,
                               int wave_slots, double advantage, uint32_t* choice, uint32_t* slots_in_use, uint32_t* colsum, uint32_t* first,
                               uint2* tasktab, hipStream_t stream);
@@ -143,7 +162,8 @@
 hipError_t prepare_spread_dense(int dtype, int M, bool poly);
 hipError_t launch_smarch_halo_add(const TileKernelArgs& a, const SMarchPlan& sp, const uint32_t* flag, hipStream_t stream);
 hipError_t launch_smarch_tasks(const Geom& g, const SMarchPlan& sp, const uint32_t* offsets, int64_t np, int cus, double advantage,
-                               uint32_t* choice, uint32_t* slots_in_use, uint32_t* colsum, uint32_t* first, uint2* tasktab, hipStream_t stream);
+                               uint32_t* choice, uint32_t* slots_in_use, uint32_t* colsum, uint32_t* first, uint2* tasktab, hipStream_t stream,
+                               RingTasks* collect = nullptr);
 
 struct GradLaunchArgs {
     int dtype, is_complex, D, M, C;
diff --git a/nonuniformffts.jl_amd/csrc/nufft_internal.h b/nonuniformffts.jl_amd/csrc/nufft_internal.h
--- a/nonuniformffts.jl_amd/csrc/nufft_internal.h
+++ b/nonuniformffts.jl_amd/csrc/nufft_internal.h
@@ -205,3 +205,5 @@
     void* ev_end[NUFFT_NUM_STAGES] = {};
     bool ev_valid[NUFFT_NUM_STAGES] = {};
 };
+
+extern "C" int nufft_internal_copy_table(nufft_plan* plan, int which, void* dst, int64_t capacity_bytes, int64_t* bytes_out, void* stream);
diff --git a/nonuniformffts.jl_amd/csrc/plan.cpp b/nonuniformffts.jl_amd/csrc/plan.cpp
--- a/nonuniformffts.jl_amd/csrc/plan.cpp
+++ b/nonuniformffts.jl_amd/csrc/plan.cpp
@@ -673,6 +673,13 @@
             p->coarse.flag_a = p->d_smarch_choice + 2;
             p->coarse.flag_b = p->d_march_choice + 2;
             if ((rc = dev_alloc(p, reinterpret_cast<void**>(&p->coarse.table), (size_t)p->coarse.groups * nkeys * sizeof(uint32_t), "sort_slice_table"))) return rc;
+            p->coarse.chain = env_int("NUFFT_SETPOINTS_CHAIN", 1) != 0 ? 1 : 0;
+            if (p->coarse.chain) {
+                const size_t words = (size_t)coarse_keyoff_words(nkeys) + 16;
+                if ((rc = dev_alloc(p, reinterpret_cast<void**>(&p->coarse.keyoff), words * sizeof(uint32_t), "sort_key_prefix"))) return rc;
+                NUFFT_HIP(hipMemset(p->coarse.keyoff, 0, words * sizeof(uint32_t)));
+                p->coarse.tickets = p->coarse.keyoff + (words - 16);
+            }
             NUFFT_HIP(prepare_binsort_coarse(p->dtype, nkeys));
             NUFFT_HIP(prepare_interp_march_staged(p->dtype, mcplx, p->M, p->evalmode != NUFFT_EVAL_DIRECT));
         }
@@ -1292,9 +1299,12 @@
         q.skip_a = coarse ? p->coarse.flag_a : nullptr;
         q.skip_b = coarse ? p->coarse.flag_b : nullptr;
         q.sp_served = coarse ? p->coarse.flag_a : nullptr;
-        NUFFT_HIP(launch_balance(q, stream));
+        if (coarse && s.cs.chain) NUFFT_HIP(launch_binsort_coarse_finish_short(s, q, stream));
+        else NUFFT_HIP(launch_balance(q, stream));
         return NUFFT_OK;
     };
+    const bool short_chain = coarse && s.cs.chain != 0;
+    RingTasks ring_a{}, ring_b{};
     if (!coarse && (rc = balance())) return rc;
     if (p->spread_method == NUFFT_SPREAD_MFMA_PATCHES) {
         PatchPlan pp{};
@@ -1316,7 +1326,7 @@
         if (p->spread_method_req == NUFFT_SPREAD_MARCHING_RING) advantage = 0.0;
         const size_t ncols = (size_t)p->smarch.ct.ncolx * p->smarch.ct.ncoly;
         NUFFT_HIP(launch_smarch_tasks(s.g, p->smarch, p->d_offsets, np, std::max(1, p->num_cus / (p->C * p->smarch.parts)), advantage, p->d_smarch_choice, p->bal.d_slots, p->d_smarch_cols,
-                                      p->d_smarch_cols + ncols, static_cast<uint2*>(p->d_smarch_tasks), stream));
+                                      p->d_smarch_cols + ncols, static_cast<uint2*>(p->d_smarch_tasks), stream, short_chain ? &ring_a : nullptr));
     }
     if (p->interp_march) {
         const double rho = (double)np / (double)std::max<int64_t>(p->grid_elems, 1), mr = (double)p->M / 4.0;
@@ -1325,10 +1335,11 @@
         const double rho_star = (0.038 * std::pow(mr, 1.85) - 0.0086 * std::pow(mr, 1.2)) / 0.09;
         const size_t ncols = (size_t)p->march_ct.ncolx * p->march_ct.ncoly;
         NUFFT_HIP(launch_march_tasks(s.g, p->march_ct, p->d_offsets, np, p->num_cus, advantage, 2.5 * rho_star, p->d_march_choice, p->d_march_cols,
-                                     p->d_march_cols + ncols, static_cast<uint2*>(p->d_march_tasks), stream));
-    }
+                                     p->d_march_cols + ncols, static_cast<uint2*>(p->d_march_tasks), stream, short_chain ? &ring_b : nullptr));
+    }
+    if (short_chain) NUFFT_HIP(launch_coarse_plan(s.g, s.cs, p->d_offsets, np, ring_a, ring_b, stream));
     if (coarse) {
-        NUFFT_HIP(launch_binsort_coarse_finish(s, stream));
+        if (!short_chain) NUFFT_HIP(launch_binsort_coarse_finish(s, stream));
         if ((rc = balance())) return rc;
     } else if (p->sort_feedback && p->coarse.enabled && !p->dense_now) {
         NUFFT_HIP(launch_sort_feedback(p->coarse.flag_a, p->coarse.flag_b, p->sort_feedback, ++p->sort_seq, stream));
@@ -1819,4 +1830,41 @@
     return NUFFT_OK;
 }
 
-}
+int nufft_internal_copy_table(nufft_plan* p, int which, void* dst, int64_t capacity_bytes, int64_t* bytes_out, void* stream_) {
+    int rc = require_points(p);
+    if (rc) return rc;
+    if (!bytes_out) return fail(NUFFT_ERR_INVALID_ARG, "null output");
+    DeviceGuard guard(p->device);
+    hipStream_t stream = static_cast<hipStream_t>(stream_);
+    const int64_t ntiles = (int64_t)p->tile.sp.ntiles + p->tile.ip.ntiles;
+    const bool ring = p->spread_method == NUFFT_SPREAD_MARCHING_RING;
+    const void* src = nullptr;
+    int64_t bytes = 0;
+    switch (which) {
+        case 0: src = p->d_offsets; bytes = ((int64_t)p->tile.nbins + 1) * 4; break;
+        case 1: if (ring) { src = p->d_smarch_tasks; bytes = (int64_t)column_task_table_entries(p->smarch.ct, p->tile.nb[2]) * 8; } break;
+        case 2: if (ring) { src = p->d_smarch_choice; bytes = 64; } break;
+        case 3: if (p->interp_march) { src = p->d_march_tasks; bytes = (int64_t)column_task_table_entries(p->march_ct, p->tile.nb[2]) * 8; } break;
+        case 4: if (p->interp_march) { src = p->d_march_choice; bytes = 64; } break;
+        case 5: src = p->bal.d_nslices; bytes = ntiles * 4; break;
+        case 6: src = p->bal.d_desc_off; bytes = (ntiles + 1) * 4; break;
+        case 7: src = p->bal.d_desc; bytes = (ntiles + p->bal.extra[0] + p->bal.extra[1]) * 8; break;
+        case 8: src = p->bal.d_slots; bytes = 8; break;
+        case 9: src = p->d_sorted; bytes = p->Np * (int64_t)point_record_bytes(p->dtype, p->D); break;
+        case 10: if (p->coarse.enabled && p->coarse.chain) { src = p->coarse.tickets; bytes = 64; } break;
+        case 11: {
+            const uint32_t geo[4] = {(uint32_t)p->tile.sp.ntiles, (uint32_t)p->tile.ip.ntiles, p->bal.extra[0], p->bal.extra[1]};
+            *bytes_out = sizeof(geo);
+            if (dst && capacity_bytes >= (int64_t)sizeof(geo)) std::memcpy(dst, geo, sizeof(geo));
+            return NUFFT_OK;
+        }
+        default: return fail(NUFFT_ERR_INVALID_ARG, "unknown table");
+    }
+    *bytes_out = src ? bytes : 0;
+    if (!src || bytes == 0 || !dst || capacity_bytes < bytes) return NUFFT_OK;
+    NUFFT_HIP(hipMemcpyAsync(dst, src, (size_t)bytes, hipMemcpyDeviceToHost, stream));
+    NUFFT_HIP(hipStreamSynchronize(stream));
+    return NUFFT_OK;
+}
+
+}
```

New measurement: 3.138 billion, median of 6. +2.0%, better.
